# pananananas/MVD

Measured on AMD Instinct MI355X. Metric: UNet forward-passes/sec @512x512 SD2.1+MV adapter, higher is better.
Workload: dtype bf16; 1 GPU; cfg4: configs[3]/[4]: 8 objects x 4 target views per GPU (32 pairs), camera FiLM + cross-view adapter; pairs_per_gpu=32, global_pairs=32, latent=64x64x4, image=512x512, forward=cold, hip_graph=False, q2_statistics=replica-local, parallelism=dp1 (pairs sharded by object), weights=synthetic seeded, SD2.1 shapes (865.9M UNet x2 + 99.2M adapter + 19.1M camera), encoder_weights=distinct

## Files before the change

include/mvd_hip.h:

```cpp
#ifndef MVD_HIP_H
#define MVD_HIP_H
#include <stddef.h>
#include <stdint.h>

#ifdef __cplusplus
extern "C" {
#endif

#define MVD_MAX_LEVELS 4

typedef struct {
  int in_channels;
  int out_channels;
  int num_levels;
  int block_out_channels[MVD_MAX_LEVELS];
  int num_heads[MVD_MAX_LEVELS];
  int layers_per_block;
  int cross_attention_dim;
  int norm_num_groups;
  float norm_eps;
  int cam_output_dim;
  int cam_hidden_dim;
  int simple_cam_encoder;
  float cam_modulation_strength;
} mvd_config_t;

typedef struct mvd_engine mvd_engine_t;

const char* mvd_last_error(void);

int mvd_engine_create(const mvd_config_t* cfg, mvd_engine_t** out);
int mvd_engine_destroy(mvd_engine_t* e);

int mvd_engine_set_weight(mvd_engine_t* e, int set, const char* slot, const void* ptr, int64_t numel, int dtype);
int mvd_engine_clear_weights(mvd_engine_t* e, int set);

int64_t mvd_engine_workspace_bytes(mvd_engine_t* e, int batch, int height, int width, int text_len, int ref_batch);
int64_t mvd_engine_refcache_bytes(mvd_engine_t* e, int ref_batch, int height, int width, int keep_features);
int mvd_engine_bind_workspace(mvd_engine_t* e, void* ws, int64_t ws_bytes, void* refcache, int64_t refcache_bytes);

enum {
  MVD_USE_CAMERA = 1,
  MVD_USE_IMAGE = 2,
  MVD_REUSE_REF = 4,
  MVD_KEEP_FEATURES = 8,
  MVD_SHARE_REF = 16,
  MVD_DEEPCACHE_REFRESH = 32,
  MVD_DEEPCACHE_SHALLOW = 64
};


typedef struct {
  int batch;
  int height, width;
  int text_len;
  const float* sample;
  const float* timesteps;
  const float* text;
  const float* source_camera;
  const float* target_camera;
  int cam_rows;
  int cam_batch;
  const float* fourier_proj;
  const float* source_latents;
  const float* encoder_text;
  int ref_batch;
  int flags;
  float* out;
// ... 22 lines not shown

int mvd_engine_set_deepcache(mvd_engine_t* e, int branch);
int mvd_engine_clear_deepcache(mvd_engine_t* e);
int64_t mvd_engine_deepcache_bytes(mvd_engine_t* e, int batch, int height, int width);
int mvd_engine_bind_deepcache(mvd_engine_t* e, void* ptr, int64_t bytes);

int mvd_engine_set_profiling(mvd_engine_t* e, int enable);
int mvd_engine_profile_summary(mvd_engine_t* e, int cap, int* cls, int* launches, double* ms, double* flops, double* bytes);
int mvd_engine_profile_shapes(mvd_engine_t* e, char* buf_host, int cap);

int mvd_engine_num_features(mvd_engine_t* e);
int mvd_engine_feature_shape(mvd_engine_t* e, int idx, int* channels, int* height, int* width);
int mvd_engine_get_feature(mvd_engine_t* e, int idx, float* out_nchw, void* stream);
int mvd_engine_encode_cameras(mvd_engine_t* e, const float* source_camera, const float* target_camera, int cam_rows,
                              int batch, const float* fourier_proj, float* out_emb, void* stream);
int mvd_engine_apply_modulation(mvd_engine_t* e, const char* name, const float* emb, int batch, const float* x_nchw,
                                int channels, int hw, float* out_nchw, void* stream);
int mvd_engine_get_camera_embedding(mvd_engine_t* e, float* out, void* stream);
int mvd_engine_film_params(mvd_engine_t* e, const float* emb, int cam_batch, int out_rows, float* out, void* stream);
int mvd_engine_time_projection(mvd_engine_t* e, const float* timesteps, int batch, float* out, void* stream);

int mvd_op_linear(const void* a, const void* a2, int k1, int k2, const void* w, const float* bias, const float* rowvec,
                  int ld_rowvec, int rows_per_batch, const void* res, float alpha, int geglu, void* out, int out_f32,
                  int m, int n, int force_cfg, int splitk, float* splitk_ws ,
                  void* stream);
int mvd_op_linear_ld(const void* a, const void* a2, int k1, int k2, const void* w, int ldw, const float* bias, const float* rowvec,
                     int ld_rowvec, int rows_per_batch, const void* res, int ldres, float alpha, int geglu, void* out, int ldo,
                     int out_f32, int m, int n, int force_cfg, int splitk, float* splitk_ws ,
                     void* stream);
int mvd_op_ln_linear(const void* x, int k, const void* w_folded, const float* c1, const float* c2, float eps, int geglu,
                     void* out, int m, int n, void* stream);
int mvd_op_linear_xs(const void* x, int ldx, const void* w_packed, int m, int k, int units, int geglu, int ln, float ln_eps,
                     const void* res, int ldres, void* out, int ldo, int csplit, void* stream);
int mvd_op_conv3x3_ws(const void* x, int batch, int h, int w, int c, const void* w_packed, const float* bias, const float* rowvec,
                      int ld_rowvec, const void* res, const void* sc, const void* sc2, int sc_c1, int sc_c2, void* out, int n,
                      int variant, void* stream);
int mvd_op_conv3x3(const void* x, int batch, int in_h, int in_w, int cin, int stride, int upsample, int asym_pad, const void* w,
                   const float* bias, const float* rowvec, int ld_rowvec, const void* res, const void* sc, const void* sc2,
                   int sc_c1, int sc_c2, void* out, int cout, int force_cfg, int splitk, float* splitk_ws, void* stream);
int mvd_op_conv3x3_up4(const void* x, int batch, int in_h, int in_w, int cin, const void* w4, const float* bias, void* out, int cout,
                       int force_cfg, void* stream);
int mvd_op_attention(const void* q, const void* k, const void* v, void* o, int batch, int heads, int nq, int nk, int ldq,
                     int ldk, int ldv, int ldo, float scale, void* stream);
int mvd_op_attention_grouped(const void* q, const void* k, const void* v, void* o, int batch, int heads, int nq, int nk, int ldq,
                             int ldk, int ldv, int ldo, float scale, int kv_group, void* stream);
int mvd_op_attention_objects(const void* q, const void* k, const void* v, void* o, int batch, int heads, int nq, int nk, int ldq,
                             int ldk, int ldv, int ldo, float scale, int kv_group, int kv_objects, void* stream);
int mvd_op_attention_mapped(const void* q, const void* k, const void* v, void* o, int batch, int heads, int nq, int nk, int ldq,
                            int ldk, int ldv, int ldo, float scale, const int* kv_index_host, int kv_elements, void* stream);
int64_t mvd_op_attention_split_ws_bytes(int batch, int heads, int nq, int nsplit);
int mvd_op_attention_split(const void* q, const void* k, const void* v, void* o, int batch, int heads, int nq, int nk, int ldq,
                           int ldk, int ldv, int ldo, int nsplit, void* ws, void* stream);
int mvd_op_groupnorm(const void* x0, const void* x1, int c0, int c1, int batch, int hw, int groups, float eps,
                     const float* gamma, const float* beta, int silu, void* y, float* ws, void* stream);
int mvd_op_layernorm(const void* x, int rows, int c, float eps, const float* gamma, const float* beta, void* y,
                     void* stream);
int mvd_op_refnorm(const void* x, int batch, int hw, int c, void* y, void* stream);
int mvd_op_refnorm_grouped(const void* x, int batch, int group, int hw, int c, void* y, void* stream);
int mvd_op_film(const void* x, int batch, int hw, int c, const float* scale, const float* shift, void* y, void* stream);
int mvd_op_conv_in(const void* x, int batch, int h, int w, int cin, const float* wt, const float* bias, int cout, void* y,
                   void* stream);
int mvd_op_conv_out(const void* x, int batch, int h, int w, int c, const void* wt, const float* bias, int cout, float* y,
                    void* stream);
int mvd_op_nchw_to_nhwc(const float* x, int batch, int c, int hw, const float* scale, const float* shift, void* y,
                        void* stream);
int mvd_op_nhwc_to_nchw(const void* x, int batch, int hw, int c, float* y, void* stream);
int mvd_op_f32_to_bf16(const float* x, int64_t n, void* y, void* stream);
int mvd_op_skinny_linear(const float* x, int ldx, int batch, int k, const void* w, int wbf16, const float* bias, int n, int act_in,
                         float* y, int ldy, void* stream);
int mvd_op_timestep_embedding(const float* t, int batch, int dim, float* y, void* stream);
int mvd_op_camera_features(const float* src, const float* tgt, int batch, int cam_rows, int nfreq, float max_freq, float* rflat,
                           float* enc, void* stream);
int mvd_op_layernorm_f32(const float* x, int rows, int c, float eps, const float* gamma, const float* beta, int silu, int nseg,
                         float* y, void* stream);
int mvd_op_skinny_linear_grouped(const float* x, int ldx, int xseg, int batch, int k, const float* w, const float* bias, int n,
                                 const int* seg_end, int nseg, float* y, int ldy, void* stream);
int mvd_op_film_params(const float* raw, int batch, int dim, float strength, float* scale, float* shift, int out_rows,
                       void* stream);
int mvd_op_film_params_grouped(const float* raw, int batch, const int* seg_end, int nseg, float strength, float* out, int out_rows,
                               void* stream);
int mvd_op_im2col_in(const float* x, int batch, int c, int h, int w, const float* scale, const float* shift, int ld_ss, void* y,
                     void* stream);
int mvd_op_film_nchw_f32(const float* x, int batch, int c, int hw, const float* scale, const float* shift, float* y, void* stream);
int mvd_gemm_num_configs(void);
int mvd_debug_last_gemm_plan(int* out);
int mvd_debug_last_attention_plan(int* out);
int mvd_debug_last_groupnorm_plan(int* out);
long mvd_debug_up4_launches(void);
int mvd_debug_last_gemm_nowait(void);
int mvd_debug_pick_splitk(int m, int n, int k, int geglu);
int mvd_debug_pick_splitk_conv(int m, int n, int k);
int mvd_debug_dense_route(int m, int n, int k1, int k2, int* out);
int mvd_debug_gemm_pp_takes(int m, int n, int k, int ldw, int ldres, int ldo);
int mvd_gemm_sm_num_tiles(void);
int mvd_debug_set_attention_nw(int nw_log2);
int mvd_debug_ragged_tables(const int* view_counts, int objects, int g, int* adapter, int* text);
// ... 17 lines not shown
int mvd_op_vit_fold(const float* x, const float* delta, int64_t n, float* out, void* stream);
int mvd_op_clip_l2norm(float* x, int rows, int dim, void* stream);
int mvd_op_vae_pointwise(const float* x, int batch, int cin, int cout, int hw, const float* w, const float* bias, float* y, void* stream);
int64_t mvd_debug_clip_linear_ws_bytes(int M, int N, int K, int out_f32);
int mvd_debug_clip_linear(const void* a, int K, int M, const void* w, const float* bias, int N, void* out, int out_f32, void* ws,
                          int64_t ws_bytes, int* route_out, void* stream);
int mvd_debug_clip_attention(const void* qkv_bf16, void* out_bf16, int batch, int heads, int tokens, void* stream);
typedef enum {
  MVD_DBG_NO_SM_LN_FOLD = 1,
  MVD_DBG_SM_NO_SPLITK = 2,
  MVD_DBG_NO_SM = 4,
  MVD_DBG_NO_SPLIT_KV = 8,
  MVD_DBG_ONE_STREAM = 16,
  MVD_DBG_SINGLE_STREAM_POLICY = 32,
  MVD_DBG_SIDE_DEFAULT_PRIORITY = 64,
  MVD_DBG_NO_XS = 128,
  MVD_DBG_NO_WS = 256,
  MVD_DBG_WS_SMALL_MAPS = 512,
  MVD_DBG_WS_BLOCK64 = 1024,
  MVD_DBG_WS_NO_SHORTCUT = 2048,
  MVD_DBG_WS_NOT_IN_ENCODER = 4096,
  MVD_DBG_WS_ONLY_IN_ENCODER = 8192,
  MVD_DBG_WS_THEN_TILED = 16384,
  MVD_DBG_WS_CHECK = 32768,
  MVD_DBG_GRAPH_ONE_STREAM = 65536,
  MVD_DBG_PP_ROW_MAJOR = 131072,
  MVD_DBG_NO_DEEP_CONV_SPLIT = 262144,
  MVD_DBG_LATE_FROM_UP1 = 524288,
  MVD_DBG_NO_UP4 = 1048576,
  MVD_DBG_GN_ONE_PASS = 2097152,
  MVD_DBG_FORK_LATE = 4194304,
  MVD_DBG_SKINNY_VECTOR = 8388608
} mvd_debug_flag_t;
int mvd_debug_set_flags(int flags);

int mvd_op_ddpm_step(const float* model_out, const float* sample, const float* noise, float c0, float c1, float c2,
                     float c3, float sigma, float* out, int64_t n, void* stream);
int mvd_op_cfg_combine(const float* uncond_cond, float guidance_scale, float* out, int64_t n_half, void* stream);
int mvd_op_sampler_step(const float* model_out, int guided, float guidance_scale, const float* sample, const float* x0_prev,
                        const float* noise, float a0, float a1, float p, float q, float r, float sigma, float* out,
                        float* x0_out, int64_t n, void* stream);
int mvd_op_cfg_rescale(const float* uncond_cond, float guidance_scale, float guidance_rescale, float* out, int64_t rows,
                       int64_t n_row, void* stream);
int mvd_op_sampler_step_rescaled(const float* model_out, float guidance_scale, float guidance_rescale, const float* sample,
                                 const float* x0_prev, const float* noise, float a0, float a1, float p, float q, float r,
                                 float sigma, float* out, float* x0_out, int64_t rows, int64_t n_row, void* stream);
int mvd_debug_cfg_rescale_plan(int64_t n_row, int* out);
int mvd_op_apg(const float* uncond_cond, float guidance_scale, float eta, float norm_threshold, float momentum,
               float guidance_rescale, float* momentum_buffer, float* out, int64_t rows, int64_t n_row, void* stream);
int mvd_op_sampler_step_apg(const float* model_out, float guidance_scale, float eta, float norm_threshold, float momentum,
                            float guidance_rescale, int space, float* momentum_buffer, const float* sample, const float* x0_prev,
                            const float* noise, float a0, float a1, float p, float q, float r, float sigma, float* out,
                            float* x0_out, int64_t rows, int64_t n_row, void* stream);
int mvd_debug_apg_plan(int64_t n_row, int* out);

int mvd_op_freeu(const void* hidden, int C, const void* skip, int Cs, int B, int H, int W, float b, float s, void* hidden_out,
                 void* skip_out, void* stream);

int mvd_op_add_noise(const float* x0, const float* noise, const int32_t* timesteps, const float* sqrt_ac, const float* sqrt_1mac,
                     int num_train_timesteps, float* noisy, float* velocity, int batch, int64_t per_sample, void* stream);
int64_t mvd_op_noise_loss_ws_bytes(int batch, int64_t per_sample);
int mvd_op_noise_loss(const float* pred, const float* noise, const float* x0, const float* noisy, const int32_t* timesteps,
                      const float* sqrt_ac, const float* sqrt_1mac, const float* snr, int num_train_timesteps, int prediction_type,
                      float snr_gamma, float* denoised, float* result, int batch, int64_t per_sample, void* ws, int64_t ws_bytes,
                      void* stream);
int64_t mvd_op_image_metrics_ws_bytes(int n, int c, int h, int w, int want_ssim);
// ... 148 lines not shown
```

mvd_amd/_lib.py:

```python
from __future__ import annotations

import ctypes as C
import enum
import os

HERE = os.path.dirname(os.path.abspath(__file__))
LIB_PATH = os.environ.get("MVD_HIP_LIB") or os.path.join(HERE, "libmvd_hip.so")

MVD_MAX_LEVELS = 4
MVD_USE_CAMERA, MVD_USE_IMAGE, MVD_REUSE_REF, MVD_KEEP_FEATURES, MVD_SHARE_REF = 1, 2, 4, 8, 16
MVD_DEEPCACHE_REFRESH, MVD_DEEPCACHE_SHALLOW = 32, 64


class MvdError(RuntimeError):
    pass


class DebugFlag(enum.IntFlag):
    NO_SM_LN_FOLD = 1
    SM_NO_SPLITK = 2
    NO_SM = 4
    NO_SPLIT_KV = 8
    ONE_STREAM = 16
    SINGLE_STREAM_POLICY = 32
# ... 34 lines not shown
        ("norm_eps", C.c_float),
    ]


class mvd_text_config_t(C.Structure):
    _fields_ = [
        ("vocab_size", C.c_int), ("hidden_size", C.c_int), ("intermediate_size", C.c_int), ("num_layers", C.c_int),
        ("num_heads", C.c_int), ("max_positions", C.c_int), ("layer_norm_eps", C.c_float), ("act", C.c_int),
    ]


class mvd_vision_config_t(C.Structure):
    _fields_ = [
        ("image_size", C.c_int), ("patch_size", C.c_int), ("hidden_size", C.c_int), ("intermediate_size", C.c_int),
        ("num_layers", C.c_int), ("num_heads", C.c_int), ("projection_dim", C.c_int), ("layer_norm_eps", C.c_float), ("act", C.c_int),
    ]


class mvd_forward_args_t(C.Structure):
    _fields_ = [
        ("batch", C.c_int), ("height", C.c_int), ("width", C.c_int), ("text_len", C.c_int),
        ("sample", C.c_void_p), ("timesteps", C.c_void_p), ("text", C.c_void_p),
        ("source_camera", C.c_void_p), ("target_camera", C.c_void_p), ("cam_rows", C.c_int), ("cam_batch", C.c_int),
        ("fourier_proj", C.c_void_p), ("source_latents", C.c_void_p), ("encoder_text", C.c_void_p),
        ("ref_batch", C.c_int), ("flags", C.c_int), ("out", C.c_void_p), ("views", C.c_int),
    ]


_SIGS = {
    "mvd_last_error": (C.c_char_p, []),
    "mvd_engine_create": (C.c_int, [C.POINTER(mvd_config_t), C.POINTER(C.c_void_p)]),
    "mvd_engine_destroy": (C.c_int, [C.c_void_p]),
    "mvd_engine_set_weight": (C.c_int, [C.c_void_p, C.c_int, C.c_char_p, C.c_void_p, C.c_int64, C.c_int]),
    "mvd_engine_clear_weights": (C.c_int, [C.c_void_p, C.c_int]),
    "mvd_engine_workspace_bytes": (C.c_int64, [C.c_void_p, C.c_int, C.c_int, C.c_int, C.c_int, C.c_int]),
    "mvd_engine_workspace_bytes_args": (C.c_int64, [C.c_void_p, C.POINTER(mvd_forward_args_t)]),
    "mvd_engine_workspace_bytes_objects": (C.c_int64, [C.c_void_p, C.POINTER(mvd_forward_args_t), C.c_int]),
    "mvd_engine_refcache_bytes": (C.c_int64, [C.c_void_p, C.c_int, C.c_int, C.c_int, C.c_int]),
    "mvd_engine_bind_workspace": (C.c_int, [C.c_void_p, C.c_void_p, C.c_int64, C.c_void_p, C.c_int64]),
    "mvd_unet_forward": (C.c_int, [C.c_void_p, C.POINTER(mvd_forward_args_t), C.c_void_p]),
    "mvd_unet_forward_objects": (C.c_int, [C.c_void_p, C.POINTER(mvd_forward_args_t), C.c_int, C.c_void_p]),
    "mvd_unet_forward_ragged": (C.c_int, [C.c_void_p, C.POINTER(mvd_forward_args_t), C.POINTER(C.c_int), C.c_int, C.c_void_p]),
    "mvd_engine_workspace_bytes_ragged": (C.c_int64, [C.c_void_p, C.POINTER(mvd_forward_args_t), C.POINTER(C.c_int), C.c_int]),
    "mvd_debug_ragged_tables": (C.c_int, [C.POINTER(C.c_int), C.c_int, C.c_int, C.POINTER(C.c_int), C.POINTER(C.c_int)]),
    "mvd_engine_set_profiling": (C.c_int, [C.c_void_p, C.c_int]),
    "mvd_engine_profile_summary": (C.c_int, [C.c_void_p, C.c_int, C.POINTER(C.c_int), C.POINTER(C.c_int),
                                             C.POINTER(C.c_double), C.POINTER(C.c_double), C.POINTER(C.c_double)]),
    "mvd_engine_profile_shapes": (C.c_int, [C.c_void_p, C.c_char_p, C.c_int]),
    "mvd_engine_set_graph": (C.c_int, [C.c_void_p, C.c_int]),
    "mvd_engine_reference_pixels": (C.c_int64, [C.c_void_p, C.c_int, C.c_int]),
    "mvd_engine_reference_encode": (C.c_int, [C.c_void_p, C.POINTER(mvd_forward_args_t), C.c_void_p, C.c_void_p]),
    "mvd_engine_reference_finish": (C.c_int, [C.c_void_p, C.c_void_p, C.c_void_p]),
    "mvd_engine_share_encoder_weights": (C.c_int, [C.c_void_p, C.c_int]),
    "mvd_engine_num_features": (C.c_int, [C.c_void_p]),
    "mvd_engine_feature_shape": (C.c_int, [C.c_void_p, C.c_int, C.POINTER(C.c_int), C.POINTER(C.c_int), C.POINTER(C.c_int)]),
    "mvd_engine_get_feature": (C.c_int, [C.c_void_p, C.c_int, C.c_void_p, C.c_void_p]),
    "mvd_engine_encode_cameras": (C.c_int, [C.c_void_p, C.c_void_p, C.c_void_p, C.c_int, C.c_int, C.c_void_p, C.c_void_p, C.c_void_p]),
    "mvd_engine_apply_modulation": (C.c_int, [C.c_void_p, C.c_char_p, C.c_void_p, C.c_int, C.c_void_p, C.c_int, C.c_int, C.c_void_p, C.c_void_p]),
    "mvd_engine_get_camera_embedding": (C.c_int, [C.c_void_p, C.c_void_p, C.c_void_p]),
    "mvd_engine_film_params": (C.c_int, [C.c_void_p, C.c_void_p, C.c_int, C.c_int, C.c_void_p, C.c_void_p]),
    "mvd_engine_time_projection": (C.c_int, [C.c_void_p, C.c_void_p, C.c_int, C.c_void_p, C.c_void_p]),
    "mvd_op_linear": (C.c_int, [C.c_void_p, C.c_void_p, C.c_int, C.c_int, C.c_void_p, C.c_void_p, C.c_void_p, C.c_int,
                                C.c_int, C.c_void_p, C.c_float, C.c_int, C.c_void_p, C.c_int, C.c_int, C.c_int, C.c_int,
                                C.c_int, C.c_void_p, C.c_void_p]),
    "mvd_op_linear_ld": (C.c_int, [C.c_void_p, C.c_void_p, C.c_int, C.c_int, C.c_void_p, C.c_int, C.c_void_p, C.c_void_p, C.c_int,
                                   C.c_int, C.c_void_p, C.c_int, C.c_float, C.c_int, C.c_void_p, C.c_int, C.c_int, C.c_int, C.c_int,
                                   C.c_int, C.c_int, C.c_void_p, C.c_void_p]),
    "mvd_op_ln_linear": (C.c_int, [C.c_void_p, C.c_int, C.c_void_p, C.c_void_p, C.c_void_p, C.c_float, C.c_int, C.c_void_p,
                                   C.c_int, C.c_int, C.c_void_p]),
    "mvd_op_linear_xs": (C.c_int, [C.c_void_p, C.c_int, C.c_void_p, C.c_int, C.c_int, C.c_int, C.c_int, C.c_int, C.c_float,
                                   C.c_void_p, C.c_int, C.c_void_p, C.c_int, C.c_int, C.c_void_p]),
    "mvd_op_conv3x3_ws": (C.c_int, [C.c_void_p, C.c_int, C.c_int, C.c_int, C.c_int, C.c_void_p, C.c_void_p, C.c_void_p, C.c_int,
                                    C.c_void_p, C.c_void_p, C.c_void_p, C.c_int, C.c_int, C.c_void_p, C.c_int, C.c_int, C.c_void_p]),
    "mvd_op_conv3x3": (C.c_int, [C.c_void_p, C.c_int, C.c_int, C.c_int, C.c_int, C.c_int, C.c_int, C.c_int, C.c_void_p, C.c_void_p,
                                 C.c_void_p, C.c_int, C.c_void_p, C.c_void_p, C.c_void_p, C.c_int, C.c_int, C.c_void_p,
                                 C.c_int, C.c_int, C.c_int, C.c_void_p, C.c_void_p]),
    "mvd_op_attention": (C.c_int, [C.c_void_p, C.c_void_p, C.c_void_p, C.c_void_p, C.c_int, C.c_int, C.c_int, C.c_int,
                                   C.c_int, C.c_int, C.c_int, C.c_int, C.c_float, C.c_void_p]),
    "mvd_op_attention_grouped": (C.c_int, [C.c_void_p, C.c_void_p, C.c_void_p, C.c_void_p, C.c_int, C.c_int, C.c_int, C.c_int,
                                           C.c_int, C.c_int, C.c_int, C.c_int, C.c_float, C.c_int, C.c_void_p]),
    "mvd_op_attention_objects": (C.c_int, [C.c_void_p, C.c_void_p, C.c_void_p, C.c_void_p, C.c_int, C.c_int, C.c_int, C.c_int,
                                           C.c_int, C.c_int, C.c_int, C.c_int, C.c_float, C.c_int, C.c_int, C.c_void_p]),
    "mvd_op_attention_mapped": (C.c_int, [C.c_void_p, C.c_void_p, C.c_void_p, C.c_void_p, C.c_int, C.c_int, C.c_int, C.c_int,
                                          C.c_int, C.c_int, C.c_int, C.c_int, C.c_float, C.POINTER(C.c_int), C.c_int, C.c_void_p]),
    "mvd_debug_attention_mapped_grouped": (C.c_int, [C.c_void_p, C.c_void_p, C.c_void_p, C.c_void_p, C.c_int, C.c_int, C.c_int, C.c_int,
                                                     C.c_int, C.c_int, C.c_int, C.c_int, C.c_float, C.c_int, C.c_int, C.POINTER(C.c_int),
                                                     C.c_int, C.c_void_p]),
    "mvd_debug_attention_pair_ws_bytes": (C.c_int64, [C.POINTER(C.c_int), C.POINTER(C.c_int), C.POINTER(C.c_int), C.c_int, C.c_int,
                                                      C.c_float, C.c_int]),
    "mvd_debug_attention_pair": (C.c_int, [C.POINTER(C.c_void_p), C.POINTER(C.c_int), C.POINTER(C.c_int), C.POINTER(C.c_int), C.c_int,
                                           C.c_int, C.c_float, C.c_int, C.c_void_p, C.c_void_p]),
    "mvd_op_attention_split_ws_bytes": (C.c_int64, [C.c_int, C.c_int, C.c_int, C.c_int]),
    "mvd_op_attention_split": (C.c_int, [C.c_void_p, C.c_void_p, C.c_void_p, C.c_void_p, C.c_int, C.c_int, C.c_int, C.c_int, C.c_int,
                                         C.c_int, C.c_int, C.c_int, C.c_int, C.c_void_p, C.c_void_p]),
    "mvd_op_groupnorm": (C.c_int, [C.c_void_p, C.c_void_p, C.c_int, C.c_int, C.c_int, C.c_int, C.c_int, C.c_float,
                                   C.c_void_p, C.c_void_p, C.c_int, C.c_void_p, C.c_void_p, C.c_void_p]),
    "mvd_op_layernorm": (C.c_int, [C.c_void_p, C.c_int, C.c_int, C.c_float, C.c_void_p, C.c_void_p, C.c_void_p, C.c_void_p]),
    "mvd_op_refnorm": (C.c_int, [C.c_void_p, C.c_int, C.c_int, C.c_int, C.c_void_p, C.c_void_p]),
    "mvd_op_refnorm_grouped": (C.c_int, [C.c_void_p, C.c_int, C.c_int, C.c_int, C.c_int, C.c_void_p, C.c_void_p]),
    "mvd_op_film": (C.c_int, [C.c_void_p, C.c_int, C.c_int, C.c_int, C.c_void_p, C.c_void_p, C.c_void_p, C.c_void_p]),
    "mvd_op_conv_in": (C.c_int, [C.c_void_p, C.c_int, C.c_int, C.c_int, C.c_int, C.c_void_p, C.c_void_p, C.c_int, C.c_void_p, C.c_void_p]),
    "mvd_op_conv_out": (C.c_int, [C.c_void_p, C.c_int, C.c_int, C.c_int, C.c_int, C.c_void_p, C.c_void_p, C.c_int, C.c_void_p, C.c_void_p]),
    "mvd_op_nchw_to_nhwc": (C.c_int, [C.c_void_p, C.c_int, C.c_int, C.c_int, C.c_void_p, C.c_void_p, C.c_void_p, C.c_void_p]),
    "mvd_op_nhwc_to_nchw": (C.c_int, [C.c_void_p, C.c_int, C.c_int, C.c_int, C.c_void_p, C.c_void_p]),
    "mvd_op_f32_to_bf16": (C.c_int, [C.c_void_p, C.c_int64, C.c_void_p, C.c_void_p]),
    "mvd_op_skinny_linear": (C.c_int, [C.c_void_p, C.c_int, C.c_int, C.c_int, C.c_void_p, C.c_int, C.c_void_p, C.c_int, C.c_int,
                                        C.c_void_p, C.c_int, C.c_void_p]),
    "mvd_op_timestep_embedding": (C.c_int, [C.c_void_p, C.c_int, C.c_int, C.c_void_p, C.c_void_p]),
    "mvd_op_camera_features": (C.c_int, [C.c_void_p, C.c_void_p, C.c_int, C.c_int, C.c_int, C.c_float, C.c_void_p, C.c_void_p, C.c_void_p]),
    "mvd_op_layernorm_f32": (C.c_int, [C.c_void_p, C.c_int, C.c_int, C.c_float, C.c_void_p, C.c_void_p, C.c_int, C.c_int, C.c_void_p,
                                       C.c_void_p]),
    "mvd_op_skinny_linear_grouped": (C.c_int, [C.c_void_p, C.c_int, C.c_int, C.c_int, C.c_int, C.c_void_p, C.c_void_p, C.c_int,
                                               C.POINTER(C.c_int), C.c_int, C.c_void_p, C.c_int, C.c_void_p]),
    "mvd_op_film_params": (C.c_int, [C.c_void_p, C.c_int, C.c_int, C.c_float, C.c_void_p, C.c_void_p, C.c_int, C.c_void_p]),
    "mvd_op_film_params_grouped": (C.c_int, [C.c_void_p, C.c_int, C.POINTER(C.c_int), C.c_int, C.c_float, C.c_void_p, C.c_int, C.c_void_p]),
    "mvd_op_im2col_in": (C.c_int, [C.c_void_p, C.c_int, C.c_int, C.c_int, C.c_int, C.c_void_p, C.c_void_p, C.c_int, C.c_void_p, C.c_void_p]),
    "mvd_op_film_nchw_f32": (C.c_int, [C.c_void_p, C.c_int, C.c_int, C.c_int, C.c_void_p, C.c_void_p, C.c_void_p, C.c_void_p]),
    "mvd_gemm_num_configs": (C.c_int, []),
    "mvd_debug_last_gemm_plan": (C.c_int, [C.POINTER(C.c_int)]),
    "mvd_debug_up4_launches": (C.c_long, []),
    "mvd_op_conv3x3_up4": (C.c_int, [C.c_void_p, C.c_int, C.c_int, C.c_int, C.c_int, C.c_void_p, C.c_void_p, C.c_void_p, C.c_int, C.c_int,
                                     C.c_void_p]),
    "mvd_debug_last_gemm_nowait": (C.c_int, []),
    "mvd_debug_last_attention_plan": (C.c_int, [C.POINTER(C.c_int)]),
    "mvd_debug_last_groupnorm_plan": (C.c_int, [C.POINTER(C.c_int)]),
    "mvd_debug_pick_splitk": (C.c_int, [C.c_int, C.c_int, C.c_int, C.c_int]),
    "mvd_debug_pick_splitk_conv": (C.c_int, [C.c_int, C.c_int, C.c_int]),
    "mvd_debug_dense_route": (C.c_int, [C.c_int, C.c_int, C.c_int, C.c_int, C.POINTER(C.c_int)]),
    "mvd_debug_gemm_pp_takes": (C.c_int, [C.c_int, C.c_int, C.c_int, C.c_int, C.c_int, C.c_int]),
    "mvd_gemm_sm_num_tiles": (C.c_int, []),
    "mvd_debug_set_attention_nw": (C.c_int, [C.c_int]),
    "mvd_debug_set_flags": (C.c_int, [C.c_int]),
    "mvd_op_ddpm_step": (C.c_int, [C.c_void_p, C.c_void_p, C.c_void_p, C.c_float, C.c_float, C.c_float, C.c_float,
                                   C.c_float, C.c_void_p, C.c_int64, C.c_void_p]),
# ... 224 lines not shown
```

mvd_amd/csrc/engine.hip:

```cpp
#include <math.h>
#include <stdio.h>
#include <stdlib.h>
#include <string.h>

#include <mutex>
#include <string>
#include <unordered_map>
#include <vector>

#include "host_util.h"
#include "ragged.h"

int mvd_launch_silu_to_bf16(const float* x, int64_t n, bf16_t* y, hipStream_t s);

static int g_debug_flags = 0;
extern "C" int mvd_debug_set_flags(int flags) { g_debug_flags = flags; return 0; }
int mvd_debug_flags() { return g_debug_flags; }

namespace {

struct FeatureInfo { std::string name; int level; int C; int heads; std::string key;  };
constexpr int MVD_REF_ONLY_INTERNAL = 1 << 30;

}
// ... 7 lines not shown
  std::vector<FeatureInfo> feats;
  std::vector<bf16_t*> refkv;
  std::vector<bf16_t*> feat_keep;
  int rc_batch = 0, rc_h = 0, rc_w = 0; bool rc_valid = false; bool rc_keep = false;
  std::vector<int> rc_layout;
  float* ref_stats_out = nullptr;
  bool rc_pending = false;
  int64_t ref_pixels(int h, int w) const { int64_t n = 0; for (auto& f : feats) n += (int64_t)(h >> f.level) * (w >> f.level); return n; }
  int64_t feat_pixel_off(int idx) const { int64_t n = 0; for (int i = 0; i < idx; ++i) n += (int64_t)(rc_h >> feats[i].level) * (rc_w >> feats[i].level); return n; }
  float* cam_emb = nullptr; int cam_batch = 0;
  unsigned int* cnt_base = nullptr; int cnt_used = 0, cnt_cap = 0;
  hipStream_t side = nullptr;
  std::vector<hipEvent_t> feat_ev;
  hipEvent_t fork_ev = nullptr, join_ev = nullptr;
  bool dual_now = false;
  int ensure_side_stream() {
    if (side) return 0;
    {
      int lo = 0, hi = 0;
      (void)hipDeviceGetStreamPriorityRange(&lo, &hi);
      const int pr = (g_debug_flags & MVD_DBG_SIDE_DEFAULT_PRIORITY) ? 0 : hi;
      if (hipStreamCreateWithPriority(&side, hipStreamNonBlocking, pr) != hipSuccess) { mvd_set_error("engine: hipStreamCreate failed"); return -3; }
    }
    feat_ev.resize(feats.size());
    for (auto& ev : feat_ev) if (hipEventCreateWithFlags(&ev, hipEventDisableTiming) != hipSuccess) { mvd_set_error("engine: hipEventCreate failed"); return -3; }
    if (hipEventCreateWithFlags(&fork_ev, hipEventDisableTiming) != hipSuccess || hipEventCreateWithFlags(&join_ev, hipEventDisableTiming) != hipSuccess) { mvd_set_error("engine: hipEventCreate failed"); return -3; }
    return 0;
  }
  bool share_encoder = false;
  bool freeu_on = false; float freeu_b[2] = {1.f, 1.f}, freeu_s[2] = {1.f, 1.f};
  bool dc_on = false; int dc_branch = 0;
  void* dc_ptr = nullptr; int64_t dc_bytes = 0;
  uint64_t weight_gen = 0;
  struct DeepRecord { bool valid = false; int batch = 0, h = 0, w = 0, cam = 0, img = 0, branch = 0; uint64_t wgen = 0; std::vector<int> layout; } dc_rec;
  bool dc_sizing = false;
  int dc_hidden_channels() const { return cfg.layers_per_block - 1 - dc_branch >= 1 ? cfg.block_out_channels[0] : cfg.block_out_channels[1]; }
  struct HostState {
    std::vector<bf16_t*> refkv, feat_keep;
    int rc_batch, rc_h, rc_w; bool rc_valid, rc_keep;
    float* cam_emb; int cam_batch;
    std::vector<int> rc_layout;
  };
  HostState host_state() const { return {refkv, feat_keep, rc_batch, rc_h, rc_w, rc_valid, rc_keep, cam_emb, cam_batch, rc_layout}; }
  void set_host_state(const HostState& h) {
    refkv = h.refkv; feat_keep = h.feat_keep; rc_batch = h.rc_batch; rc_h = h.rc_h; rc_w = h.rc_w; rc_valid = h.rc_valid;
    rc_keep = h.rc_keep; cam_emb = h.cam_emb; cam_batch = h.cam_batch; rc_layout = h.rc_layout;
  }
  struct GraphEntry { std::string key; hipGraph_t g; hipGraphExec_t x; HostState after; };
  bool dual_late = false;
  bool graph_on = false;
  std::vector<GraphEntry> graphs;
  std::vector<std::string> graph_seen;
  void drop_graphs() {
    for (auto& ge : graphs) { (void)hipGraphExecDestroy(ge.x); (void)hipGraphDestroy(ge.g); }
    graphs.clear(); graph_seen.clear();
  }
  struct KvSlot { std::vector<int> layout , host ; int* dev = nullptr; uint64_t used = 0; };
  static constexpr size_t KV_SLOTS = 8;
  std::vector<KvSlot> kv_slots; uint64_t kv_tick = 0;
  ~mvd_engine() {
    drop_graphs();
    for (auto& sl : kv_slots) if (sl.dev) (void)hipFree(sl.dev);
    for (hipEvent_t ev : ev_pool) (void)hipEventDestroy(ev);
    for (hipEvent_t ev : feat_ev) if (ev) (void)hipEventDestroy(ev);
    if (fork_ev) (void)hipEventDestroy(fork_ev);
    if (join_ev) (void)hipEventDestroy(join_ev);
    if (side) (void)hipStreamDestroy(side);
  }
  std::vector<int> temb_off;
  int temb_total = 0;
  std::vector<int> tkv_off;
  int tkv_total = 0;
  bool prof = false;
  bool prof_overlap = false;
  struct ProfRec { int cls; double flops; double bytes; hipEvent_t e0, e1; int M, N, K, tag; };
  int prof_M = 0, prof_N = 0, prof_K = 0, prof_tag = 0;
  std::vector<ProfRec> prof_recs;
  std::vector<hipEvent_t> ev_pool; size_t ev_used = 0;
  hipEvent_t get_event() {
    if (ev_used == ev_pool.size()) { hipEvent_t ev = nullptr; (void)hipEventCreate(&ev); ev_pool.push_back(ev); }
    return ev_pool[ev_used++];
  }
};

static inline int gemm_class(const MvdGemmArgs& g, int cfg, int splitk) {
  if (cfg == 8) return MVD_PC_GEMM_128X320;
  if (cfg == 7) return splitk > 1 ? MVD_PC_PP_SPLITK : (g.seg[0].mode == MVD_A_CONV3 ? MVD_PC_PP_CONV3 : (g.ln_c1 ? MVD_PC_PP_LN_DENSE : MVD_PC_PP_DENSE));
  return MVD_PC_GEMM_256X160 + cfg;
}
int mvd_attention_pick_nw(const MvdAttnArgs& a);

namespace {

#ifdef MVD_PROBE
struct WsCheckRec { std::string slot; int set; bool side; const char* p[4]; size_t n[4]; };
// ... 107 lines not shown
      if (sm_S > 1) {
        g.splitk = sm_S; g.splitk_nowait = nowait ? 1 : 0; g.part = talloc<float>((size_t)sm_S * g.M * g.N);
        const int tiles = ((g.M + 63) / 64) * (g.N / 64);
        g.tile_cnt = e->cnt_base + e->cnt_used;
        e->cnt_used += tiles;
        if (!dry && e->cnt_used > e->cnt_cap) { mvd_set_error("forward: split-K tile counters exhausted (%d > %d)", e->cnt_used, e->cnt_cap); return err = -15; }
      }
      int r = 0;
      if (!dry) {
        const double fl = 2.0 * g.M * (double)g.N * g.Ktot;
        e->prof_M = g.M; e->prof_N = g.N; e->prof_K = g.Ktot; e->prof_tag = (tag_base >= 0 ? tag_base : g.seg[0].mode * 100 + g.geglu * 10) + (sm_S > 1 ? sm_S : 0);
        r = profiled(MVD_PC_SM_64X64 + sm_tile, fl, 0.0, [&] { return mvd_launch_gemm_sm(g, s, sm_tile, sm_ns); });
      }
      e->tmp.off = mark;
      return r;
    }
    int S = 1, fc = -1;
    tiled_plan(g, S, fc);
    const size_t mark = e->tmp.off;
    if (S > 1) { g.splitk = S; g.part = talloc<float>((size_t)S * g.M * g.N); } else g.splitk = 1;
    static const bool trace = MVD_ENV_INT("MVD_TRACE_GEMM", 0) != 0;
    if (trace && !dry) fprintf(stderr, "gemm M=%d N=%d K=%d mode=%d nseg=%d geglu=%d cfg=%d splitk=%d\n", g.M, g.N, g.Ktot, g.seg[0].mode, g.nseg, g.geglu, mvd_gemm_pick_config(g), S);
    int r = 0;
    if (!dry) {
      const double fl = 2.0 * g.M * (double)g.N * g.Ktot;
      e->prof_M = g.M; e->prof_N = g.N; e->prof_K = g.Ktot; e->prof_tag = (tag_base >= 0 ? tag_base : g.seg[0].mode * 100 + g.geglu * 10) + (S > 1 ? S : 0);
      r = launch_tiled(g, s, fc, [&](auto&& launch) { return profiled(e->prof ? gemm_class(g, mvd_gemm_pick_config(g), S) : 0, fl, 0.0, launch); });
    }
    e->tmp.off = mark;
    return r;
  }

  int try_xs(const bf16_t* x, int K, int M, const std::string& slot, int64_t n_full, int N, bool geglu, bool ln,
             const bf16_t* res, int ldres, void* out, int ldo, int set_override = -1) {
    if (err) return err;
    if (dry || (g_debug_flags & MVD_DBG_NO_XS) || K != 320 || slot.empty() || !has(slot, set_override)) return 0;
    MvdXsArgs a; memset(&a, 0, sizeof(a));
    a.x = x; a.ldx = K; a.M = M; a.K = K; a.units = N / 32; a.geglu = geglu; a.ln = ln; a.ln_eps = 1e-5f;
    a.res = res; a.ldres = ldres; a.out = (bf16_t*)out; a.ldo = ldo;
    if (N % 64 || !mvd_gemm_xs_applicable(a)) return 0;
    if ((long)((M + 255) / 256) * mvd_gemm_xs_pick_csplit(a) < 448) return 0;
    a.w = WB(slot, (n_full / 32) * 21 * 512, set_override);
    if (!a.w) return err;
    e->prof_M = M; e->prof_N = N; e->prof_K = K; e->prof_tag = geglu * 10 + (ln ? 1 : 0);
    const int r = profiled(geglu ? MVD_PC_XS_GEGLU : (res ? MVD_PC_XS_RESIDUAL : (ln ? MVD_PC_XS_LN_DENSE : MVD_PC_XS_DENSE)), 2.0 * M * (double)N * K, 0.0, [&] { return mvd_launch_gemm_xs(a, s); });
    return r ? r : 1;
  }

  int linear(const bf16_t* a, const bf16_t* a2, int k1, int k2, int M, const bf16_t* w, const float* bias, int N,
             const bf16_t* res, int ldres, void* out, int ldo, bool geglu = false, bool out_f32 = false, int ldw = 0,
             const std::string& xs = std::string(), int xs_set = -1) {
    if (!xs.empty() && !a2 && !k2 && !geglu && !out_f32) {
      const int r = try_xs(a, k1, M, xs, N, N, false, false, res, ldres, out, ldo, xs_set);
      if (r) return r < 0 ? r : 0;
    }
    MvdGemmArgs g = gemm_dense(a, a2, k1, k2, M, w, ldw, bias, N, out, ldo);
    g.res = res; g.ldres = ldres; g.geglu = geglu; g.out_f32 = out_f32;
    return gemm(g);
  }

  int ln_linear(const bf16_t* x, int M, int C, const std::string& ln_key, const std::string& slot, int64_t n_full, int N,
                const float* bias, bf16_t* ln_tmp, void* out, int ldo, bool geglu) {
    MvdGemmArgs g = gemm_dense(x, nullptr, C, 0, M, nullptr, 0, nullptr, N, out, ldo);
    g.geglu = geglu;
    {
      const int r = try_xs(x, C, M, slot + ".wx", n_full, N, geglu, true, nullptr, 0, out, ldo);
      if (r) return r < 0 ? r : 0;
    }
    static const bool use_fold = MVD_ENV_INT("MVD_LN_FOLD", 1) != 0;
    auto sm_fold_ok = [&]() {
      MvdGemmArgs t = g;
      static const float dummy = 0.f;
      t.ln_c1 = &dummy; t.bias = &dummy; t.W = reinterpret_cast<const bf16_t*>(&dummy);
      int a_, b_, c_;
      return sm_enabled() && !(g_debug_flags & MVD_DBG_NO_SM_LN_FOLD) && mvd_gemm_sm_plan(t, &a_, &b_, &c_);
    };
// ... 248 lines not shown
      const bf16_t* kv2 = tkv + c.e->tkv_off[feat_idx];
      const int ldkv = c.e->tkv_total;
      CHECK(c.ln_linear(h, M, C, key + ".ln2", key + ".attn2.q", (int64_t)(packed ? 2 : 1) * C, nq, nullptr, ln, q2, nq, false));
      MvdAttnArgs a; memset(&a, 0, sizeof(a));
      a.batch = B_; a.heads = heads; a.scale = scale; a.prescaled = 1; a.nprob = ad ? 2 : 1;
      a.p[0] = {q2, kv2, kv2 + C, o_self, nq, ldkv, ldkv, C, (int64_t)hw * nq, (int64_t)L * ldkv, (int64_t)L * ldkv, (int64_t)hw * C, hw, L};
      if (ad) a.p[1] = {q2 + C, rkv + 2 * C, rkv + 3 * C, o_ref, nq, 4 * C, 4 * C, C, (int64_t)hw * nq, (int64_t)ref_nk * 4 * C, (int64_t)ref_nk * 4 * C, (int64_t)hw * C, hw, ref_nk};
      if (ad) o.layout->fill_map(false, &a.kv_group[0], &a.kv_objects[0], &a.kv_index[0]);
      if (ad) o.layout->fill_map(true, &a.kv_group[1], &a.kv_objects[1], &a.kv_index[1]);
      CHECK(c.attention(a));
      CHECK(c.linear(o_self, o_ref, C, ad ? C : 0, M, c.WB(key + ".attn2.out.w", (int64_t)C * ld_out), c.WF(key + ".attn2" + bias_slot, C), C, h, C, h, C, false, false, ld_out,
                     ad ? std::string() : key + ".attn2.out.wx"));
    }
    {
      bf16_t* ff = c.talloc<bf16_t>((size_t)M * 4 * C);
      CHECK(c.ln_linear(h, M, C, key + ".ln3", key + ".ff1", (int64_t)8 * C, 8 * C, c.WF(key + ".ff1.b", 8 * C), ln, ff, 4 * C, true));
      const bool tail = c.has(key + ".tail.w");
      if (tail || c.dry) {
        c.tag_base = 50;
        const int r = c.linear(ff, h, 4 * C, C, M, c.WB(key + ".tail.w", (int64_t)C * 5 * C), c.WF(key + ".tail.b", C), C, x.p, C, out.p, C);
        c.tag_base = -1;
        CHECK(r);
      }
      if (!tail) {
        CHECK(c.linear(ff, nullptr, 4 * C, 0, M, c.WB(key + ".ff2.w", (int64_t)C * 4 * C), c.WF(key + ".ff2.b", C), C, h, C, h, C));
        CHECK(c.linear(h, nullptr, C, 0, M, c.WB(key + ".proj_out.w", (int64_t)C * C), c.WF(key + ".proj_out.b", C), C, x.p, C, out.p, C, false, false, 0, key + ".proj_out.wx"));
      }
    }
    c.e->tmp.off = mark;

    if (o.capture) {
      const size_t mk = c.e->tmp.off;
      bf16_t* rn = c.talloc<bf16_t>((size_t)M * C);
      if (o.defer_norm) {
        if (!c.dry && !c.err) CHECK(mvd_launch_refstats(out.p, B_, hw, C, o.stats + 2 * c.e->feat_pixel_off(feat_idx), c.s));
      } else {
        if (!c.dry && !c.err) CHECK(o.layout->per_object_stats() ? mvd_launch_refnorm_grouped(out.p, B_, 1, hw, C, rn, c.s) : mvd_launch_refnorm(out.p, B_, hw, C, rn, c.s));
        CHECK(c.linear(rn, nullptr, C, 0, M, c.WB(key + ".ref_kv.w", (int64_t)4 * C * C, 0), nullptr, 4 * C, nullptr, 0, c.e->refkv[feat_idx], 4 * C, false, false, 0,
                       key + ".ref_kv.wx", 0));
        if (c.e->dual_now && !c.dry && !c.err && hipEventRecord(c.e->feat_ev[feat_idx], c.s) != hipSuccess) { mvd_set_error("forward: hipEventRecord failed"); return -3; }
      }
      if (c.e->rc_keep && !c.dry && !c.err)
        CHECK((int)hipMemcpyAsync(c.e->feat_keep[feat_idx], out.p, (size_t)M * C * sizeof(bf16_t), hipMemcpyDeviceToDevice, c.s));
      c.e->tmp.off = mk;
    }
    ++feat_idx;
    return c.err;
  }

  int film(const std::string& name, const Act& x, Act& out) {
    auto it = o.film_ss->find(name);
    if (it == o.film_ss->end()) { out = x; return 0; }
    if (c.dry || c.err) return c.err;
    return mvd_launch_film(x.p, x.B, x.hw(), x.C, it->second.first, it->second.second, x.C, out.p, c.s);
  }

  int down_resnet_pos(int i, int j) const { return i * cfg.layers_per_block + j; }
  int mid_resnet_pos(int j) const { return cfg.num_levels * cfg.layers_per_block + j; }
  int up_resnet_pos(int i, int j) const { return cfg.num_levels * cfg.layers_per_block + 2 + i * (cfg.layers_per_block + 1) + j; }
  int down_feat_pos(int i, int j) const { return i * cfg.layers_per_block + j; }
  int mid_feat_pos() const { return (cfg.num_levels - 1) * cfg.layers_per_block; }
  int up_feat_pos(int i, int j) const { return (cfg.num_levels - 1) * cfg.layers_per_block + 1 + (i - 1) * (cfg.layers_per_block + 1) + j; }

  int run(const Act& x_in, float* out_nchw) {
    const int n = cfg.num_levels, Lb = cfg.layers_per_block;
    const int C0 = cfg.block_out_channels[0];
    const bool shallow = o.deep == MVD_DEEPCACHE_SHALLOW, refresh = o.deep == MVD_DEEPCACHE_REFRESH;
    const int j0 = Lb - 1 - o.deep_branch;
    std::vector<Act> skips;
    const int TB = text_rows > 0 ? text_rows : B;
    tkv = c.aalloc<bf16_t>((size_t)TB * L * c.e->tkv_total);
    CHECK(c.linear(text, nullptr, cfg.cross_attention_dim, 0, TB * L, c.WB("text_kv.w", (int64_t)c.e->tkv_total * cfg.cross_attention_dim), nullptr,
// ... 57 lines not shown
        if (refresh && i == n - 1 && j == j0 && !c.dry && !c.err)
          CHECK((int)hipMemcpyAsync(o.deep_buf, h.p, (size_t)h.rows() * h.C * sizeof(bf16_t), hipMemcpyDeviceToDevice, c.s));
        Act r = c.new_act(B, h.H, h.W, co, true);
        resnet_idx = up_resnet_pos(i, j);
        if (o.freeu && i < 2) {
          const size_t fm = c.e->tmp.off;
          Act hf = c.new_act(B, h.H, h.W, h.C, false), sf = c.new_act(B, skip.H, skip.W, skip.C, false);
          if (!c.dry && !c.err) CHECK(mvd_launch_freeu(h.p, h.C, skip.p, skip.C, B, h.H, h.W, c.e->freeu_b[i], c.e->freeu_s[i], hf.p, sf.p, c.s));
          CHECK(resnet(bk + ".resnets." + std::to_string(j), hf, &sf, co, r));
          c.e->tmp.off = fm;
        } else {
          CHECK(resnet(bk + ".resnets." + std::to_string(j), h, &skip, co, r));
        }
        h = r;
        if (i > 0) {
          Act t = c.new_act(B, h.H, h.W, co, true);
          feat_idx = up_feat_pos(i, j);
          CHECK(transformer(bk + ".attentions." + std::to_string(j), h, cfg.num_heads[n - 1 - i], t));
          h = t;
        }
      }
      if (i + 1 < n) {
        Act u = c.new_act(B, h.H * 2, h.W * 2, co, true);
        CHECK(c.conv3(h, 1, 1, c.WB(bk + ".up.w", (int64_t)co * 9 * co), c.WF(bk + ".up.b", co), nullptr, 0, nullptr, nullptr, nullptr, 0, 0, u, bk + ".up.ws", bk + ".up.w4"));
        h = u;
      }
      if (o.film) { Act res = h; CHECK(film("up_" + std::to_string(i), h, res)); h = res; }
    }
    if (out_nchw) {
      Act t = c.new_act(B, h.H, h.W, C0, false);
      CHECK(c.groupnorm(h.p, nullptr, C0, 0, B, h.hw(), cfg.norm_eps, c.WF("conv_norm_out.g", C0), c.WF("conv_norm_out.b", C0), 1, t.p));
      const bf16_t* wo = c.WB("conv_out.w", (int64_t)cfg.out_channels * 9 * C0);
      const float* bo = c.WF("conv_out.b", cfg.out_channels);
      if (!c.dry && !c.err) CHECK(mvd_launch_conv_out(t.p, B, h.H, h.W, C0, wo, bo, cfg.out_channels, out_nchw, c.s));
    }
    return c.err;
  }
};

int time_path(Ctx& c, const float* timesteps, int B, const float** tproj_out) {
  const mvd_config_t& cfg = c.e->cfg;
  const int C0 = cfg.block_out_channels[0], TD = 4 * C0;
  float* sinus = c.talloc<float>((size_t)B * C0);
  float* t1 = c.talloc<float>((size_t)B * TD);
  float* emb = c.talloc<float>((size_t)B * TD);
  bf16_t* act = c.talloc<bf16_t>((size_t)B * TD);
  float* tproj = c.aalloc<float>((size_t)B * c.e->temb_total);
  const bf16_t* w1 = c.WB("time.l1.w", (int64_t)TD * C0);
  const float* b1 = c.WF("time.l1.b", TD);
  const bf16_t* w2 = c.WB("time.l2.w", (int64_t)TD * TD);
  const float* b2 = c.WF("time.l2.b", TD);
  const bf16_t* wp = c.WB("temb_proj.w", (int64_t)c.e->temb_total * TD);
  const float* bp = c.WF("temb_proj.b", c.e->temb_total);
  *tproj_out = tproj;
  if (c.err) return c.err;
  if (c.dry) return 0;
  CHECK(mvd_launch_timestep_embedding(timesteps, B, C0, sinus, c.s));
  CHECK(mvd_launch_skinny_linear(sinus, C0, B, C0, w1, 1, b1, TD, 0, t1, TD, c.s));
  CHECK(mvd_launch_skinny_linear(t1, TD, B, TD, w2, 1, b2, TD, 1, emb, TD, c.s));
  CHECK(mvd_launch_silu_to_bf16(emb, (int64_t)B * TD, act, c.s));
  CHECK(c.linear(act, nullptr, TD, 0, B, wp, bp, c.e->temb_total, nullptr, 0, tproj, c.e->temb_total, false, true));
  return 0;
}

int camera_embed(Ctx& c, const float* src, const float* tgt, int cam_rows, const float* proj, int B, float* emb) {
  const mvd_config_t& cfg = c.e->cfg;
  const int D = cfg.cam_output_dim, Hd = cfg.cam_hidden_dim;
  const int nfreq = (D / 2) / 3, encd = 6 * nfreq;
  const bool simple = cfg.simple_cam_encoder != 0;
  float* rflat = c.talloc<float>((size_t)B * 9);
  float* enc = c.talloc<float>((size_t)B * encd);
  float* encp = c.talloc<float>((size_t)B * D);
  float* cat = c.talloc<float>((size_t)B * 2 * D);
  float* bufa = c.talloc<float>((size_t)B * (D > Hd ? D : Hd));
  float* bufb = c.talloc<float>((size_t)B * (D > Hd ? D : Hd));
  auto lin = [&](const std::string& k, const float* x, int ldx, int kin, int nout, float* y, int ldy) -> int {
    const float* w = c.WF("cam." + k + ".weight", (int64_t)nout * kin, 0);
    const float* b = c.WF("cam." + k + ".bias", nout, 0);
    if (c.err) return c.err; if (c.dry) return 0;
    return mvd_launch_skinny_linear(x, ldx, B, kin, w, 0, b, nout, 0, y, ldy, c.s);
  };
  auto lnorm = [&](const std::string& k, const float* x, int n, int silu, float* y) -> int {
    const float* g = c.WF("cam." + k + ".weight", n, 0);
    const float* b = c.WF("cam." + k + ".bias", n, 0);
    if (c.err) return c.err; if (c.dry) return 0;
    return mvd_launch_layernorm_f32(x, B, n, 1e-5f, g, b, silu, y, c.s);
  };
  if (!c.dry && !c.err) {
    CHECK(mvd_launch_camera_features(src, tgt, B, cam_rows, nfreq, 10.0f, rflat, enc, c.s));
    CHECK(mvd_launch_skinny_linear(enc, encd, B, encd, proj, 0, nullptr, D, 0, encp, D, c.s));
  }
  const char* encs[2] = {"rotation_encoder", "translation_encoder"};
  for (int t = 0; t < 2; ++t) {
    const std::string p = encs[t];
// ... 178 lines not shown
      for (size_t i = 0; i < e->feats.size(); ++i) {
        const int lv = e->feats[i].level;
        const size_t hw = (size_t)(H >> lv) * (Wd >> lv);
        e->refkv[i] = (bf16_t*)e->persist.alloc((size_t)a.ref_batch * hw * 4 * e->feats[i].C * sizeof(bf16_t));
        if (keep) e->feat_keep[i] = (bf16_t*)e->persist.alloc((size_t)a.ref_batch * hw * e->feats[i].C * sizeof(bf16_t));
      }
      if (e->persist.overflow()) { mvd_set_error("forward: reference cache too small (%zu > %zu bytes)", e->persist.high, e->persist.cap); return -4; }
      e->rc_keep = keep; e->rc_batch = a.ref_batch; e->rc_h = H; e->rc_w = Wd; e->rc_layout = lay.key();
      if (!dry) { e->rc_valid = false; e->rc_pending = false; }
    }
  }

  const bool dual = use_img && !reuse && !ref_only;
  e->dual_late = false;
  e->dual_now = dual && !dry && !(e->graph_on && (g_debug_flags & MVD_DBG_GRAPH_ONE_STREAM)) && (!e->prof || e->prof_overlap) && !(g_debug_flags & MVD_DBG_ONE_STREAM);
  const bool early = dual && (g_debug_flags & MVD_DBG_FORK_LATE);
  auto fork = [&]() -> int {
    if (!e->dual_now) return 0;
    CHECK(e->ensure_side_stream());
    if (hipEventRecord(e->fork_ev, s) != hipSuccess || hipStreamWaitEvent(e->side, e->fork_ev, 0) != hipSuccess) { mvd_set_error("forward: stream fork failed"); return -3; }
    return 0;
  };
  if (!early) CHECK(fork());

  std::unordered_map<std::string, std::pair<float*, float*>> film_ss;
  if (use_cam) CHECK(camera_path(c, a, film_ss));
  const float* tproj_main = nullptr;
  const float* tproj_enc = nullptr;
  if (early) {
    c.set = 0;
    CHECK(time_path(c, a.timesteps, B, &tproj_main));
    c.set = e->share_encoder ? 0 : 1;
    float* tz = c.aalloc<float>(a.ref_batch);
    if (!dry) CHECK((int)hipMemsetAsync(tz, 0, a.ref_batch * sizeof(float), s));
    CHECK(time_path(c, tz, a.ref_batch, &tproj_enc));
    c.set = 0;
    CHECK(fork());
  }

  if (use_img && !reuse) {
    if (dual) e->tmp.off = e->tmp.high;
    const size_t tm = e->tmp.off, am = e->act.off;
    if (e->dual_now) { c.s = e->side; c.nowait = true; }
    c.set = e->share_encoder ? 0 : 1;
    const int Br = a.ref_batch;
    const float* tproj = tproj_enc;
    if (!tproj) {
      float* tz = c.talloc<float>(Br);
      if (!dry) CHECK((int)hipMemsetAsync(tz, 0, Br * sizeof(float), c.s));
      CHECK(time_path(c, tz, Br, &tproj));
    }
    bf16_t* tx = c.aalloc<bf16_t>((size_t)Br * L * xd);
    Act xin = c.new_act(Br, H, Wd, 64, true);
    if (!dry && !c.err) {
      CHECK(mvd_launch_f32_to_bf16(a.encoder_text, (int64_t)Br * L * xd, tx, c.s));
      CHECK(mvd_launch_im2col_in(a.source_latents, Br, cfg.in_channels, H, Wd, nullptr, nullptr, 0, xin.p, c.s));
    }
    PassOpts po; po.capture = true; po.ref_batch = Br; po.layout = &lay;
    po.defer_norm = ref_only; po.stats = e->ref_stats_out;
    UNetPass pass{c, cfg, po, Br, H, Wd, L, tx, tproj};
    CHECK(pass.run(xin, nullptr));
    if (!dry) { e->rc_valid = !ref_only; e->rc_pending = ref_only; }
    if (dual) {
      e->tmp.off = e->tmp.high;
      if (e->dual_now && hipEventRecord(e->join_ev, e->side) != hipSuccess) { mvd_set_error("forward: hipEventRecord failed"); return -3; }
      c.s = s; c.nowait = false;
    } else {
      e->tmp.off = tm; e->act.off = am;
    }
  }
  if (ref_only) {
    if (c.err) return c.err;
    if (!dry && (e->tmp.high + e->act.high > (size_t)e->ws_bytes)) { mvd_set_error("reference_encode: workspace too small"); return -4; }
    return 0;
  }

  c.set = 0;
  const float* tproj = tproj_main;
  if (!tproj) CHECK(time_path(c, a.timesteps, B, &tproj));
  const int TB = lay.text_rows(B);
  bf16_t* tx = c.aalloc<bf16_t>((size_t)TB * L * xd);
  Act xin = c.new_act(B, H, Wd, 64, true);
  if (!dry && !c.err) {
// ... 61 lines not shown
}

extern "C" {

int mvd_engine_create(const mvd_config_t* cfg, mvd_engine_t** out) {
  if (!cfg || !out) { mvd_set_error("engine_create: null argument"); return -1; }
  if (cfg->num_levels < 2 || cfg->num_levels > MVD_MAX_LEVELS || cfg->layers_per_block < 1) { mvd_set_error("engine_create: unsupported topology"); return -1; }
  for (int i = 0; i < cfg->num_levels; ++i) {
    const int c = cfg->block_out_channels[i];
    if (c % 64 || c % cfg->norm_num_groups || cfg->num_heads[i] * 64 != c) { mvd_set_error("engine_create: level %d: channels %d must be a multiple of 64/groups with head_dim 64 (heads %d)", i, c, cfg->num_heads[i]); return -1; }
  }
  if (cfg->cross_attention_dim % 64) { mvd_set_error("engine_create: cross_attention_dim must be a multiple of 64"); return -1; }
  if (cfg->in_channels > 7 || cfg->out_channels > 8) { mvd_set_error("engine_create: in_channels must be <= 7 (9*Cin <= 64) and out_channels <= 8"); return -1; }
  mvd_engine* e = new mvd_engine();
  e->cfg = *cfg;
  e->feats = enumerate_features(*cfg);
  int off = 0;
  for (auto& r : enumerate_resnets(*cfg)) { e->temb_off.push_back(off); off += r.cout; }
  e->temb_total = off;
  off = 0;
  for (auto& f : e->feats) { e->tkv_off.push_back(off); off += 2 * f.C; }
  e->tkv_total = off;
  *out = e;
  return 0;
}

int mvd_engine_destroy(mvd_engine_t* e) { delete e; return 0; }

int mvd_engine_set_weight(mvd_engine_t* e, int set, const char* slot, const void* ptr, int64_t numel, int dtype) {
  if (e) e->drop_graphs();
  if (!e || set < 0 || set > 1 || !slot || !ptr || numel <= 0 || dtype < 0 || dtype > 1) { mvd_set_error("set_weight: bad argument"); return -1; }
  if ((uintptr_t)ptr & 15) { mvd_set_error("set_weight: '%s' must be 16-byte aligned", slot); return -1; }
  e->w[set].m[slot] = Weight{ptr, numel, dtype};
  ++e->weight_gen;
  return 0;
}
int mvd_engine_clear_weights(mvd_engine_t* e, int set) {
  if (e) e->drop_graphs();
  if (!e || set < 0 || set > 1) { mvd_set_error("clear_weights: bad argument"); return -1; }
  e->w[set].m.clear();
  ++e->weight_gen;
  return 0;
}

static void fill_dry_args(mvd_forward_args_t& a, int batch, int h, int w, int L, int ref_batch) {
  memset(&a, 0, sizeof(a));
  a.batch = batch; a.height = h; a.width = w; a.text_len = L; a.ref_batch = ref_batch; a.cam_rows = 4;
  a.flags = MVD_USE_CAMERA | (ref_batch > 0 ? MVD_USE_IMAGE : 0);
}

int64_t mvd_engine_workspace_bytes(mvd_engine_t* e, int batch, int height, int width, int text_len, int ref_batch) {
  if (!e) { mvd_set_error("workspace_bytes: null engine"); return -1; }
  mvd_forward_args_t a; fill_dry_args(a, batch, height, width, text_len, ref_batch);
  const mvd_engine::HostState before = e->host_state();
  int r = forward_impl(e, a, nullptr, true);
  e->set_host_state(before);
  if (r) return r;
  return (int64_t)(((e->act.high + 255) & ~size_t(255)) + e->tmp.high + 4096);
}

static ViewLayout uniform_layout(const mvd_forward_args_t* args, int objects) {
  return args ? ViewLayout::uniform(objects, args->views, args->flags & MVD_SHARE_REF) : ViewLayout();
}

static int64_t workspace_bytes_args(mvd_engine_t* e, const mvd_forward_args_t* args, const ViewLayout& lay) {
  if (!e || !args) { mvd_set_error("workspace_bytes_args: null argument"); return -1; }
// ... 662 lines not shown
  mvd_ragged_build_tables(view_counts, objects, g, adapter, text);
  if (mvd_attention_check_index(adapter, g * R, g * objects) || mvd_attention_check_index(text, g * R, g * objects)) return -1;
  return g * R;
}

int mvd_op_attention_split(const void* q, const void* k, const void* v, void* o, int batch, int heads, int nq, int nk, int ldq,
                           int ldk, int ldv, int ldo, int nsplit, void* ws, void* stream) {
  MvdAttnArgs a; memset(&a, 0, sizeof(a));
  a.nprob = 1; a.batch = batch; a.heads = heads; a.scale = 0.f; a.prescaled = 1;
  a.p[0] = {(const bf16_t*)q, (const bf16_t*)k, (const bf16_t*)v, (bf16_t*)o, ldq, ldk, ldv, ldo,
            (int64_t)nq * ldq, (int64_t)nk * ldk, (int64_t)nk * ldv, (int64_t)nq * ldo, nq, nk};
  if (nsplit > 1) {
    if (!ws) { mvd_set_error("op_attention_split: null workspace"); return -1; }
    const size_t pb = (mvd_attention_split_ws_bytes(a, nsplit) + 255) & ~size_t(255);
    a.nsplit = nsplit; a.split_ws = ws; a.split_cnt = reinterpret_cast<unsigned int*>(reinterpret_cast<char*>(ws) + pb);
    if (hipMemsetAsync(a.split_cnt, 0, (size_t)mvd_attention_split_counters(a) * 4, (hipStream_t)stream) != hipSuccess) { mvd_set_error("op_attention_split: hipMemsetAsync failed"); return -3; }
  }
  return mvd_launch_attention(a, (hipStream_t)stream);
}

int mvd_op_groupnorm(const void* x0, const void* x1, int c0, int c1, int batch, int hw, int groups, float eps,
                     const float* gamma, const float* beta, int silu, void* y, float* ws, void* stream) {
  return mvd_launch_groupnorm((const bf16_t*)x0, (const bf16_t*)x1, c0, c1, batch, hw, groups, eps, gamma, beta, silu, (bf16_t*)y, ws, (hipStream_t)stream);
}
int mvd_op_layernorm(const void* x, int rows, int c, float eps, const float* gamma, const float* beta, void* y, void* stream) {
  return mvd_launch_layernorm((const bf16_t*)x, rows, c, eps, gamma, beta, (bf16_t*)y, (hipStream_t)stream);
}
int mvd_op_refnorm(const void* x, int batch, int hw, int c, void* y, void* stream) {
  return mvd_launch_refnorm((const bf16_t*)x, batch, hw, c, (bf16_t*)y, (hipStream_t)stream);
}
int mvd_op_refnorm_grouped(const void* x, int batch, int group, int hw, int c, void* y, void* stream) {
  return mvd_launch_refnorm_grouped((const bf16_t*)x, batch, group, hw, c, (bf16_t*)y, (hipStream_t)stream);
}
int mvd_op_film(const void* x, int batch, int hw, int c, const float* scale, const float* shift, void* y, void* stream) {
  return mvd_launch_film((const bf16_t*)x, batch, hw, c, scale, shift, c, (bf16_t*)y, (hipStream_t)stream);
}
int mvd_op_conv_in(const void* x, int batch, int h, int w, int cin, const float* wt, const float* bias, int cout, void* y, void* stream) {
  return mvd_launch_conv_in((const bf16_t*)x, batch, h, w, cin, wt, bias, cout, (bf16_t*)y, (hipStream_t)stream);
}
int mvd_op_conv_out(const void* x, int batch, int h, int w, int c, const void* wt, const float* bias, int cout, float* y, void* stream) {
  return mvd_launch_conv_out((const bf16_t*)x, batch, h, w, c, (const bf16_t*)wt, bias, cout, y, (hipStream_t)stream);
}
int mvd_op_nchw_to_nhwc(const float* x, int batch, int c, int hw, const float* scale, const float* shift, void* y, void* stream) {
  return mvd_launch_nchw_to_nhwc(x, batch, c, hw, scale, shift, c, (bf16_t*)y, (hipStream_t)stream);
}
int mvd_op_nhwc_to_nchw(const void* x, int batch, int hw, int c, float* y, void* stream) {
  return mvd_launch_nhwc_to_nchw_f32((const bf16_t*)x, batch, hw, c, y, (hipStream_t)stream);
}
int mvd_op_f32_to_bf16(const float* x, int64_t n, void* y, void* stream) {
  return mvd_launch_f32_to_bf16(x, n, (bf16_t*)y, (hipStream_t)stream);
}
int mvd_op_skinny_linear(const float* x, int ldx, int batch, int k, const void* w, int wbf16, const float* bias, int n, int act_in,
                         float* y, int ldy, void* stream) {
  return mvd_launch_skinny_linear(x, ldx, batch, k, w, wbf16, bias, n, act_in, y, ldy, (hipStream_t)stream);
}
int mvd_op_timestep_embedding(const float* t, int batch, int dim, float* y, void* stream) {
  return mvd_launch_timestep_embedding(t, batch, dim, y, (hipStream_t)stream);
}
int mvd_op_camera_features(const float* src, const float* tgt, int batch, int cam_rows, int nfreq, float max_freq, float* rflat, float* enc,
                           void* stream) {
  return mvd_launch_camera_features(src, tgt, batch, cam_rows, nfreq, max_freq, rflat, enc, (hipStream_t)stream);
}
int mvd_op_layernorm_f32(const float* x, int rows, int c, float eps, const float* gamma, const float* beta, int silu, int nseg, float* y,
                         void* stream) {
  return mvd_launch_layernorm_f32(x, rows, c, eps, gamma, beta, silu, y, (hipStream_t)stream, nseg);
}
static int op_seg_table(const int* seg_end, int nseg, MvdSegTable* seg, const char* what) {
  if (!seg_end || nseg < 1 || nseg > 16) { mvd_set_error("%s: 1..16 segment ends", what); return -1; }
  memset(seg, 0, sizeof(*seg));
  seg->n = nseg;
  for (int g = 0; g < nseg; ++g) {
// ... 30 lines not shown
```

mvd_amd/csrc/gemm_xs.hip:

```cpp
#include <stdio.h>
#include <stdlib.h>
#include <string.h>
#include "../../include/mvd_hip.h"
#include "kernels.h"
#include "bufaddr.h"

namespace {

#define XS_WAIT_VM(n) asm volatile("s_waitcnt vmcnt(" #n ")" ::: "memory")

template <int KS, bool GEGLU, bool RES, bool LN>
__global__ __launch_bounds__(256, 2) void gemm_xs_kernel(const MvdXsArgs a) {
  constexpr int NW = 4, RT = 2, NS = GEGLU ? 2 : 3;
  constexpr int STG = GEGLU ? 8192 : 4096;
  constexpr int UNIT = (KS + 1) * 1024;
  constexpr int P = KS / NW;
  static_assert(KS % NW == 0 && !(GEGLU && RES) && !(RES && LN), "shape of the instantiations");
  constexpr int E = 2 * RT + (RES ? 2 * RT : 0);
  extern __shared__ __attribute__((aligned(16))) unsigned char smem[];
  const int lane = threadIdx.x & 63;
  const int wave = __builtin_amdgcn_readfirstlane(threadIdx.x >> 6);
  const int r = lane & 31, h = lane >> 5;
#ifdef XS_DBG
  constexpr int dbg = XS_DBG;
#else
  constexpr int dbg = 0;
#endif

  int rb, cp;
  if (a.csplit == 1) { rb = blockIdx.x; cp = 0; }
  else {
    const int per = 8 * a.csplit, g = blockIdx.x / per, rem = blockIdx.x - g * per;
    rb = g * 8 + (rem & 7); cp = rem >> 3;
  }
  if (rb * 256 >= a.M) return;
  const int upp = a.units / a.csplit;
  const int u0 = cp * upp, nit = upp;
  const int row_w = rb * 256 + wave * (RT * 32);

  const __amdgpu_buffer_rsrc_t rs_w = buf_rsrc(a.w, a.units * UNIT);
  auto issue_unit = [&](int it, int stage) {
    unsigned char* dst = smem + stage * UNIT;
    const unsigned so = (unsigned)(u0 + it) * (unsigned)UNIT;
    if (dbg & 4) return;
#pragma unroll
    for (int i = 0; i < P; ++i) dma16(rs_w, dst + (wave * P + i) * 1024, (unsigned)lane * 16u, so + (unsigned)((wave * P + i) * 1024));
    dma4(rs_w, dst + KS * 1024 + wave * 256, (unsigned)lane * 4u, so + (unsigned)(KS * 1024 + wave * 256));
  };
  issue_unit(0, 0);
  if (NS == 3 && nit > 1) issue_unit(1, 1);

  const __amdgpu_buffer_rsrc_t rs_x = buf_rsrc(a.x, (int)((size_t)a.M * a.ldx * 2));
  u32x4 x[RT][KS];
#pragma unroll
  for (int t = 0; t < RT; ++t) {
    const int vo = (row_w + t * 32 + r) * a.ldx * 2 + h * 16;
#pragma unroll
    for (int s = 0; s < KS; ++s) x[t][s] = (dbg & 8) ? u32x4{0x3f803f80u, 0x3f803f80u, 0x3f803f80u, 0x3f803f80u} : __builtin_amdgcn_raw_buffer_load_b128(rs_x, vo + s * 32, 0, 0);
  }
  if constexpr (LN) {
    const float invk = 1.f / (float)(KS * 16);
    const bf16x2 ones2 = __builtin_bit_cast(bf16x2, 0x3f803f80u);
#pragma unroll
    for (int t = 0; t < RT; ++t) {
      float sm = 0.f, sq = 0.f;
#pragma unroll
      for (int s = 0; s < KS; ++s) {
        const unsigned d[4] = {x[t][s].x, x[t][s].y, x[t][s].z, x[t][s].w};
#pragma unroll
        for (int e = 0; e < 4; ++e) {
          const bf16x2 v = __builtin_bit_cast(bf16x2, d[e]);
          sq = __builtin_amdgcn_fdot2_f32_bf16(v, v, sq, false);
          sm = __builtin_amdgcn_fdot2_f32_bf16(v, ones2, sm, false);
        }
      }
      sm += __shfl_xor(sm, 32); sq += __shfl_xor(sq, 32);
      const float mean = sm * invk;
      const float rstd = rsqrtf(fmaxf(sq * invk - mean * mean, 0.f) + a.ln_eps);
      const float nb = -mean * rstd;
#pragma unroll
      for (int s = 0; s < KS; ++s) {
        const unsigned d[4] = {x[t][s].x, x[t][s].y, x[t][s].z, x[t][s].w};
        x[t][s] = u32x4{pack2bf(fmaf(bflo(d[0]), rstd, nb), fmaf(bfhi(d[0]), rstd, nb)), pack2bf(fmaf(bflo(d[1]), rstd, nb), fmaf(bfhi(d[1]), rstd, nb)),
                        pack2bf(fmaf(bflo(d[2]), rstd, nb), fmaf(bfhi(d[2]), rstd, nb)), pack2bf(fmaf(bflo(d[3]), rstd, nb), fmaf(bfhi(d[3]), rstd, nb))};
      }
    }
  }
  const u32x4 one_frag = {h == 0 ? 0x3f803f80u : 0u, 0u, 0u, 0u};

  const __amdgpu_buffer_rsrc_t rs_o = buf_rsrc(a.out, (int)((size_t)a.M * a.ldo * 2));
  __amdgpu_buffer_rsrc_t rs_r = rs_o;
  if (RES) rs_r = buf_rsrc(a.res, (int)((size_t)a.M * a.ldres * 2));
  int vo_r[RT];
#pragma unroll
  for (int t = 0; t < RT; ++t) {
    vo_r[t] = RES ? (row_w + t * 32 + r) * a.ldres * 2 + h * 32 : 0;
  }

#ifdef XS_STAMPS
  long long st_acc[6] = {0, 0, 0, 0, 0, 0};
  const long long st_begin = (long long)__builtin_amdgcn_s_memtime();
  const long long st_rbegin = (long long)__builtin_amdgcn_s_memrealtime();
  long long st_t = st_begin;
#define XS_STAMP(i) do { const long long n_ = (long long)__builtin_amdgcn_s_memtime(); st_acc[i] += n_ - st_t; st_t = n_; } while (0)
#else
#define XS_STAMP(i) do {} while (0)
#endif
  float gs[16 * RT];

  auto top = [&](int it, int stage) {
    XS_STAMP(4);
    if (it == 0) XS_WAIT_VM(0);
    else if constexpr (GEGLU) { if ((it & 3) == 0) XS_WAIT_VM(8); else XS_WAIT_VM(0); }
    else if (it == nit - 1) { if (RES) XS_WAIT_VM(16); else XS_WAIT_VM(8); }
    else { if (RES) XS_WAIT_VM(22); else XS_WAIT_VM(14); }
    static_assert(P + 1 == 6 && 2 * E == (RES ? 16 : 8), "the counted waits above are written for these instantiations");
    __builtin_amdgcn_sched_barrier(0);
// ... 143 lines not shown
        f32x16 gg[RT];
        multiply(stage, gg, gs, false);
#pragma unroll
        for (int t = 0; t < RT; ++t)
#pragma unroll
          for (int q = 0; q < 16; ++q) gs[t * 16 + q] = gg[t][q];
        stage = stage == NS - 1 ? 0 : stage + 1;
      }
      {
        top(it + 1, stage);
        f32x16 acc[RT];
        multiply(stage, acc, gs, true);
#pragma unroll
        for (int t = 0; t < RT; ++t)
#pragma unroll
          for (int q = 0; q < 16; ++q) acc[t][q] *= gs[t * 16 + q];
        stage_tile((it >> 1) & 1, acc);
        if (it & 2) flush_group((u0 + it) >> 2);
        stage = stage == NS - 1 ? 0 : stage + 1;
      }
    }
  }
#ifdef XS_STAMPS
  XS_STAMP(4);
  if (wave == 0 && lane == 0) {
    asm volatile("s_waitcnt vmcnt(0)" ::: "memory");
    long long* dst = reinterpret_cast<long long*>(a.out + (size_t)a.M * a.ldo) + (size_t)blockIdx.x * 8;
    for (int i = 0; i < 5; ++i) dst[i] = st_acc[i];
    dst[5] = (long long)__builtin_amdgcn_s_memrealtime() - st_rbegin; dst[6] = (long long)__builtin_amdgcn_s_memtime() - st_begin; dst[7] = st_rbegin; (void)st_prolog;
  }
#endif
}

template <int KS, bool GEGLU, bool RES, bool LN>
int launch_xs(const MvdXsArgs& a, hipStream_t s) {
  constexpr int LDS_BYTES = (GEGLU ? 2 : 3) * (KS + 1) * 1024 + 4 * (GEGLU ? 8192 : 4096);
  static bool init[16] = {};
  int dev = 0;
  (void)hipGetDevice(&dev);
  if (!init[dev & 15]) {
    hipError_t e = hipFuncSetAttribute(reinterpret_cast<const void*>(&gemm_xs_kernel<KS, GEGLU, RES, LN>), hipFuncAttributeMaxDynamicSharedMemorySize, LDS_BYTES);
    if (e != hipSuccess) { mvd_set_error("gemm_xs: hipFuncSetAttribute: %s", hipGetErrorString(e)); return -2; }
    init[dev & 15] = true;
    if (MVD_ENV_INT("MVD_XS_TRACE", 0)) {
      int occ = -1;
      (void)hipOccupancyMaxActiveBlocksPerMultiprocessor(&occ, reinterpret_cast<const void*>(&gemm_xs_kernel<KS, GEGLU, RES, LN>), 256, LDS_BYTES);
      fprintf(stderr, "gemm_xs<%d,%d,%d,%d>: %d workgroups per CU by the occupancy query (LDS %d B)\n", KS, (int)GEGLU, (int)RES, (int)LN, occ, LDS_BYTES);
    }
  }
  const int nrb = (a.M + 255) / 256;
  const int grid = a.csplit == 1 ? nrb : ((nrb + 7) / 8) * 8 * a.csplit;
  g_mvd_last_gemm.cfg = 9; g_mvd_last_gemm.splitk = 1; g_mvd_last_gemm.tiles = nrb * a.csplit; g_mvd_last_gemm.grid = grid; g_mvd_last_gemm.per_cu = 2;
  hipLaunchKernelGGL((gemm_xs_kernel<KS, GEGLU, RES, LN>), dim3(grid), dim3(256), LDS_BYTES, s, a);
  hipError_t e = hipGetLastError();
  if (e != hipSuccess) { mvd_set_error("gemm_xs launch: %s", hipGetErrorString(e)); return -3; }
  return 0;
}

}

bool mvd_gemm_xs_applicable(const MvdXsArgs& a) {
  const size_t lim = (size_t)1 << 31;
  if (a.K != 320 || a.units <= 0 || a.M <= 0 || a.relu) return false;
  if (a.units % (a.geglu ? 4 : 2)) return false;
  if ((a.geglu || a.ln) && a.res) return false;
  if ((size_t)(a.M + 256) * a.ldx * 2 >= lim || (size_t)(a.M + 256) * a.ldo * 2 >= lim) return false;
  if (a.res && (size_t)(a.M + 256) * a.ldres * 2 >= lim) return false;
  if ((size_t)a.units * 21 * 1024 >= lim) return false;
  if ((a.ldx & 7) || (a.ldo & 7) || (a.res && (a.ldres & 7))) return false;
  return true;
}

int mvd_gemm_xs_pick_csplit(const MvdXsArgs& a) {
  const int nrb = (a.M + 255) / 256;
  const int groups = a.units / (a.geglu ? 4 : 2);
  int cs = 1;
  while (nrb * cs < 1024 && groups % (cs * 2) == 0 && groups / (cs * 2) >= 3) cs *= 2;
  return cs;
}

int mvd_launch_gemm_xs(const MvdXsArgs& a_in, hipStream_t s) {
  MvdXsArgs a = a_in;
  if (a.csplit <= 0) a.csplit = mvd_gemm_xs_pick_csplit(a);
  const int groups = a.units / (a.geglu ? 4 : 2);
  if (!mvd_gemm_xs_applicable(a) || groups % a.csplit) {
    mvd_set_error("gemm_xs: M=%d K=%d units=%d geglu=%d csplit=%d is not a shape of the X-stationary kernels", a.M, a.K, a.units, a.geglu, a.csplit);
    return -1;
  }
  if (a.geglu) return a.ln ? launch_xs<20, true, false, true>(a, s) : launch_xs<20, true, false, false>(a, s);
  if (a.res) return launch_xs<20, false, true, false>(a, s);
  return a.ln ? launch_xs<20, false, false, true>(a, s) : launch_xs<20, false, false, false>(a, s);
}

extern "C" int mvd_op_linear_xs(const void* x, int ldx, const void* w_packed, int m, int k, int units, int geglu, int ln, float ln_eps,
                                const void* res, int ldres, void* out, int ldo, int csplit, void* stream) {
  MvdXsArgs a; memset(&a, 0, sizeof(a));
  a.x = (const bf16_t*)x; a.ldx = ldx; a.w = (const bf16_t*)w_packed; a.M = m; a.K = k; a.units = units; a.geglu = geglu;
  a.ln = ln; a.ln_eps = ln_eps; a.res = (const bf16_t*)res; a.ldres = ldres; a.out = (bf16_t*)out; a.ldo = ldo; a.csplit = csplit;
  if (!x || !w_packed || !out) { mvd_set_error("mvd_op_linear_xs: null operand"); return -1; }
  return mvd_launch_gemm_xs(a, (hipStream_t)stream);
}
```

mvd_amd/csrc/kernels.h:

```cpp
#pragma once
#include <hip/hip_runtime.h>
#include <stdint.h>
#include <atomic>
#include "common.h"
#include "../../include/mvd_hip.h"

enum { MVD_A_DENSE = 0, MVD_A_CONV3 = 1 };

struct MvdASeg {
  const bf16_t* p0;
  const bf16_t* p1;
  int c0, c1;
  int mode;
  int ksize;
  int inH, inW;
  int stride;
  int ups;
  int asym;
};

struct MvdGemmArgs {
  MvdASeg seg[2];
  int nseg;
  const bf16_t* W;
// ... 22 lines not shown
  float ln_eps;
  int walk_cg;
};
static_assert(sizeof(MvdGemmArgs) == 280, "MvdGemmArgs is a kernel argument: a size change moves the hidden arguments of every GEMM kernel");

inline bool mvd_gemm_rowvec_aligned(const MvdGemmArgs& a) { return !a.rowvec || (a.ld_rowvec % 4 == 0 && ((uintptr_t)a.rowvec & 15) == 0); }
int mvd_launch_gemm(const MvdGemmArgs& a, hipStream_t s, int force_cfg = -1);
int mvd_gemm_pick_config(const MvdGemmArgs& a);
int mvd_launch_gemm_relu(const MvdGemmArgs& a, hipStream_t s, int cfg, bool glds);
int mvd_launch_splitk_reduce_relu(const MvdGemmArgs& a, hipStream_t s, int grid);
struct MvdLaunchPlan { int cfg, splitk, tiles, grid, per_cu, nowait; };
extern thread_local MvdLaunchPlan g_mvd_last_gemm;
extern std::atomic<long> g_mvd_up4_launches;
bool mvd_gemm_pp_applicable(const MvdGemmArgs& a);
bool mvd_gemm_pp_up4_applicable(const MvdGemmArgs& a);
int mvd_gemm_pp_walk(const MvdGemmArgs& a);
int mvd_debug_flags();
bool mvd_gemm_ln_fold_ok(const MvdGemmArgs& a);
int mvd_launch_gemm_pp(const MvdGemmArgs& a, hipStream_t s);
int mvd_launch_gemm_ring(const MvdGemmArgs& a, hipStream_t s);
bool mvd_gemm_sm_applicable(const MvdGemmArgs& a, int tile);
int mvd_launch_gemm_sm(const MvdGemmArgs& a, hipStream_t s, int tile, int nstage);
bool mvd_gemm_sm_plan(const MvdGemmArgs& a, int* tile, int* nstage, int* splitk);
struct MvdXsArgs {
  const bf16_t* x; int ldx;
  const bf16_t* w;
  int M, K, units;
  int geglu;
  int ln; float ln_eps;
  const bf16_t* res; int ldres;
  bf16_t* out; int ldo;
  int csplit;
  int relu;
};
bool mvd_gemm_xs_applicable(const MvdXsArgs& a);
int mvd_gemm_xs_pick_csplit(const MvdXsArgs& a);
int mvd_launch_gemm_xs(const MvdXsArgs& a, hipStream_t s);
struct MvdWsArgs {
  const bf16_t* x; int B, H, W, C;
  int ups;
  const bf16_t* sc0; const bf16_t* sc1; int scc0, scc1;
  const bf16_t* w;
  const float* bias;
  const float* rowvec; int ld_rowvec;
  const bf16_t* res; int ldres;
  bf16_t* out; int ldo;
  int M, N;
  int variant;
  int relu;
};
bool mvd_conv_ws_applicable(const MvdWsArgs& a);
size_t mvd_conv_ws_packed_elems(int C, int sc, int N);
int mvd_launch_conv_ws(const MvdWsArgs& a, hipStream_t s);
#define MVD_OP_SPLITK_COUNTERS 4096
int mvd_launch_splitk_reduce(const MvdGemmArgs& a, hipStream_t s);
int mvd_gemm_pick_splitk(const MvdGemmArgs& a);

struct MvdAttnProblem {
  const bf16_t* q; const bf16_t* k; const bf16_t* v; bf16_t* o;
  int ldq, ldk, ldv, ldo;
  int64_t bsq, bsk, bsv, bso;
  int nq, nk;
};
struct MvdAttnArgs {
  MvdAttnProblem p[2];
  int nprob;
  int batch, heads;
  float scale;
  int prescaled;
  int dbg;
  int nsplit;
  void* split_ws;
  unsigned int* split_cnt;
  int kv_group[2];
  int kv_objects[2];
  const int* kv_index[2];
};
int mvd_attention_check_index(const int* idx, int n, int elements);
int mvd_attention_pick_split(const MvdAttnArgs& a);
size_t mvd_attention_split_ws_bytes(const MvdAttnArgs& a, int nsplit);
int mvd_attention_split_counters(const MvdAttnArgs& a);
int mvd_launch_attention(const MvdAttnArgs& a, hipStream_t s);

#define MVD_GN_MAXCHUNK 256
int mvd_launch_groupnorm(const bf16_t* x0, const bf16_t* x1, int c0, int c1, int batch, int hw, int groups,
                         float eps, const float* gamma, const float* beta, int silu, bf16_t* y, float* ws,
                         hipStream_t s);
int mvd_launch_layernorm(const bf16_t* x, int rows, int c, float eps, const float* gamma, const float* beta,
                         bf16_t* y, hipStream_t s);
int mvd_launch_refnorm(const bf16_t* x, int batch, int hw, int c, bf16_t* y, hipStream_t s);
int mvd_launch_refnorm_grouped(const bf16_t* x, int batch, int group, int hw, int c, bf16_t* y, hipStream_t s);
int mvd_launch_refstats(const bf16_t* x, int batch, int hw, int c, float* stats , hipStream_t s);
int mvd_launch_refapply(const bf16_t* x, int batch, int hw, int c, const float* mean_k , bf16_t* y, hipStream_t s);

int mvd_launch_nchw_to_nhwc(const float* x, int batch, int c, int hw, const float* scale, const float* shift,
                            int ld_ss, bf16_t* y, hipStream_t s);
int mvd_launch_film(const bf16_t* x, int batch, int hw, int c, const float* scale, const float* shift, int ld_ss,
                    bf16_t* y, hipStream_t s);
int mvd_launch_freeu(const bf16_t* hidden, int C, const bf16_t* skip, int Cs, int B, int H, int W, float b, float s, bf16_t* hidden_out,
                     bf16_t* skip_out, hipStream_t stream);
int mvd_launch_conv_in(const bf16_t* x, int batch, int h, int w, int cin, const float* wt, const float* bias,
                       int cout, bf16_t* y, hipStream_t s);
int mvd_launch_conv_out(const bf16_t* x, int batch, int h, int w, int c, const bf16_t* wt, const float* bias,
                        int cout, float* y, hipStream_t s);
int mvd_launch_im2col_in(const float* x, int batch, int c, int h, int w, const float* scale, const float* shift, int ld_ss,
                         bf16_t* y, hipStream_t s);
int mvd_launch_f32_to_bf16(const float* x, int64_t n, bf16_t* y, hipStream_t s);
int mvd_launch_nhwc_to_nchw_f32(const bf16_t* x, int batch, int hw, int c, float* y, hipStream_t s);
int mvd_launch_maxpool2x2(const bf16_t* x, int batch, int h, int w, int c, bf16_t* y, hipStream_t s);

int mvd_launch_skinny_linear(const float* x, int ldx, int batch, int k, const void* w, int wbf16, const float* bias,
                             int n, int act_in, float* y, int ldy, hipStream_t s);
struct MvdSegTable { int n; int end[16]; };
int mvd_launch_skinny_linear_grouped(const float* x, int ldx, int xseg, int batch, int k, const float* w, const float* bias, int n,
                                     const MvdSegTable& seg, float* y, int ldy, hipStream_t s);
int mvd_launch_film_params_grouped(const float* raw, int batch, const MvdSegTable& seg, float strength, float* out, int out_rows,
                                   hipStream_t s);
int mvd_launch_layernorm_f32(const float* x, int rows, int c, float eps, const float* gamma, const float* beta,
                             int silu, float* y, hipStream_t s, int nseg = 1);
int mvd_launch_timestep_embedding(const float* t, int batch, int dim, float* y, hipStream_t s);
int mvd_launch_camera_features(const float* src, const float* tgt, int batch, int cam_rows, int nfreq,
                               float max_freq, float* rflat, float* enc, hipStream_t s);
int mvd_launch_film_params(const float* raw, int batch, int dim, float strength, float* scale, float* shift, int out_rows,
                           hipStream_t s);

int mvd_launch_film_nchw_f32(const float* x, int batch, int c, int hw, const float* scale, const float* shift, float* y,
                             hipStream_t s);

void mvd_set_error(const char* fmt, ...);

enum MvdProfClass {
  MVD_PC_GEMM_256X160 = 0, MVD_PC_GEMM_256X128 = 1, MVD_PC_GEMM_128X160 = 2, MVD_PC_GEMM_128X128 = 3, MVD_PC_GEMM_128X64 = 4,
  MVD_PC_GEMM_64X64 = 5,
  MVD_PC_PP_GEGLU = 6, MVD_PC_PP_DENSE = 7,
  MVD_PC_ATTN_1WAVE = 8, MVD_PC_ATTN_2WAVE = 9, MVD_PC_ATTN_4WAVE = 10, MVD_PC_ATTN_8WAVE = 11,
// ... 9 lines not shown
```

mvd_amd/csrc/misc.hip:

```cpp
#include <stdarg.h>
#include <stdio.h>
#include <stdlib.h>
#include "host_util.h"

static thread_local char g_err[512] = "";
void mvd_set_error(const char* fmt, ...) {
  va_list ap;
  va_start(ap, fmt);
  vsnprintf(g_err, sizeof(g_err), fmt, ap);
  va_end(ap);
}
extern "C" const char* mvd_last_error(void) { return g_err; }

namespace {

__global__ void nchw_to_nhwc_kernel(const float* __restrict__ x, int c, int hw, const float* __restrict__ scale,
                                    const float* __restrict__ shift, int ld_ss, bf16_t* __restrict__ y, long total) {
  const long i = (long)blockIdx.x * blockDim.x + threadIdx.x;
  if (i >= total) return;
  const int ch = i % c;
  const long bp = i / c;
  const int p = bp % hw;
  const int b = bp / hw;
  float v = x[((size_t)b * c + ch) * hw + p];
  if (scale) v = v * scale[(size_t)b * ld_ss + ch] + shift[(size_t)b * ld_ss + ch];
  y[i] = f2bf(v);
}

__global__ void nhwc_to_nchw_f32_kernel(const bf16_t* __restrict__ x, int hw, int c, float* __restrict__ y, long total) {
  const long i = (long)blockIdx.x * blockDim.x + threadIdx.x;
  if (i >= total) return;
  const int p = i % hw;
  const long bc = i / hw;
  const int ch = bc % c;
  const int b = bc / c;
  y[i] = bf2f(x[((size_t)b * hw + p) * c + ch]);
// ... 52 lines not shown
  const long pix = (long)blockIdx.x * 4 + (threadIdx.x >> 6);
  const int hw = h * w;
  if (pix >= (long)batch * hw) return;
  const int b = pix / hw, p = pix % hw;
  const int oy = p / w, ox = p % w;
  const int vec = c >> 3;
  float acc[8];
#pragma unroll
  for (int j = 0; j < 8; ++j) acc[j] = 0.f;
  for (int q = lane; q < 9 * vec; q += 64) {
    const int tap = q / vec, v = q % vec;
    const int iy = oy + tap / 3 - 1, ix = ox + tap % 3 - 1;
    if ((unsigned)iy >= (unsigned)h || (unsigned)ix >= (unsigned)w) continue;
    const u32x4 xv = *reinterpret_cast<const u32x4*>(x + ((size_t)b * hw + iy * w + ix) * c + v * 8);
#pragma unroll
    for (int co = 0; co < 8; ++co) {
      if (co < cout) {
        const u32x4 wv = *reinterpret_cast<const u32x4*>(wt + ((size_t)co * 9 + tap) * c + v * 8);
        float a = acc[co];
#pragma unroll
        for (int j = 0; j < 4; ++j) {
          a = fmaf(bflo(xv[j]), bflo(wv[j]), a);
          a = fmaf(bfhi(xv[j]), bfhi(wv[j]), a);
        }
        acc[co] = a;
      }
    }
  }
#pragma unroll
  for (int co = 0; co < 8; ++co) {
    if (co < cout) {
      const float t = wave_sum(acc[co]);
      if (lane == 0) y[((size_t)b * cout + co) * hw + p] = t + bias[co];
    }
  }
}

__global__ void f32_to_bf16_kernel(const float* __restrict__ x, long n, bf16_t* __restrict__ y) {
  for (long i = (long)blockIdx.x * blockDim.x + threadIdx.x; i < n; i += (long)gridDim.x * blockDim.x) y[i] = f2bf(x[i]);
}

template <bool WBF16>
__global__ __launch_bounds__(256) void skinny_linear_kernel(const float* __restrict__ x, int ldx, int batch, int k,
                                                             const void* __restrict__ wv, const float* __restrict__ bias,
                                                             int n, int act_in, float* __restrict__ y, int ldy) {
  constexpr int BC = 32;
  const int lane = threadIdx.x & 63;
  const int o = blockIdx.x * 4 + (threadIdx.x >> 6);
  if (o >= n) return;
  const bool vec = !WBF16 && (k & 3) == 0 && (ldx & 3) == 0;
  for (int b0 = 0; b0 < batch; b0 += BC) {
    float acc[BC];
#pragma unroll
    for (int j = 0; j < BC; ++j) acc[j] = 0.f;
    if (vec) {
      const float* wr = reinterpret_cast<const float*>(wv) + (size_t)o * k;
      for (int kk = lane * 4; kk < k; kk += 256) {
        const f32x4 w4 = *reinterpret_cast<const f32x4*>(wr + kk);
#pragma unroll
        for (int j = 0; j < BC; ++j) {
          if (b0 + j < batch) {
            f32x4 x4 = *reinterpret_cast<const f32x4*>(x + (size_t)(b0 + j) * ldx + kk);
            if (act_in == 1) { x4[0] = silu_f(x4[0]); x4[1] = silu_f(x4[1]); x4[2] = silu_f(x4[2]); x4[3] = silu_f(x4[3]); }
            acc[j] = fmaf(x4[0], w4[0], fmaf(x4[1], w4[1], fmaf(x4[2], w4[2], fmaf(x4[3], w4[3], acc[j]))));
          }
        }
// ... 324 lines not shown
      hipLaunchKernelGGL(word_sum_kernel, dim3(1024), dim3(256), 0, s, reinterpret_cast<const unsigned*>(y), (long)on, dsum + 1);
      hipLaunchKernelGGL(word_sum_kernel, dim3(1024), dim3(256), 0, s, reinterpret_cast<const unsigned*>(y1), (long)on, dsum + 2);
      unsigned long long hs[3] = {0, 0, 0};
      (void)hipMemcpyAsync(hs, dsum, sizeof(hs), hipMemcpyDeviceToHost, s);
      (void)hipStreamSynchronize(s);
      fprintf(stderr, "conv_out hash pid %d: input %016llx  out(4-pixel) %016llx  out(1-pixel, same input) %016llx\n", (int)getpid(), hs[0], hs[1], hs[2]);
    }
    if (MVD_ENV_INT("MVD_CONV_OUT_CMP", 0)) {
      static unsigned long long* cnt = nullptr; static float* yb = nullptr; static float* yr = nullptr; static size_t yn = 0;
      static unsigned long long seen[3] = {0, 0, 0}; static int calls = 0;
      const size_t on = (size_t)batch * cout * h * w;
      if (!cnt) { (void)hipHostMalloc(&cnt, 4 * sizeof(unsigned long long), hipHostMallocMapped); cnt[0] = cnt[1] = cnt[2] = cnt[3] = 0; }
      if (yn < on) { if (yb) { (void)hipFree(yb); (void)hipFree(yr); } (void)hipMalloc(&yb, on * sizeof(float)); (void)hipMalloc(&yr, on * sizeof(float)); yn = on; }
      hipLaunchKernelGGL(conv_out4_kernel, dim3(nblk(quads, 4)), dim3(256), 0, s, x, batch, h, w, c, wt, bias, cout, yb);
      hipLaunchKernelGGL(conv_out_kernel, dim3(nblk((long)batch * h * w, 4)), dim3(256), 0, s, x, batch, h, w, c, wt, bias, cout, yr);
      hipLaunchKernelGGL(conv_out_cmp_kernel, dim3(256), dim3(256), 0, s, y, yb, yr, (long)on, 1e-3f, cnt);
      ++calls;
      volatile unsigned long long* vc = cnt;
      const unsigned long long c0 = vc[0], c1 = vc[1], c2 = vc[2];
      if (c0 != seen[0] || c1 != seen[1] || c2 != seen[2] || calls == 2 || calls == 20) {
        seen[0] = c0; seen[1] = c1; seen[2] = c2;
        fprintf(stderr, "conv_out cmp pid %d after ~%d calls: first!=second %llu  |first-ref|>1e-3 %llu  |second-ref|>1e-3 %llu  last idx %llu (x mod 4 = %llu)\n",
                (int)getpid(), calls - 1, c0, c1, c2, (unsigned long long)vc[3], (unsigned long long)vc[3] % 4);
      }
    }
    return launch_check("conv_out4");
  }
#endif
  const long pix = (long)batch * h * w;
  hipLaunchKernelGGL(conv_out_kernel, dim3(nblk(pix, 4)), dim3(256), 0, s, x, batch, h, w, c, wt, bias, cout, y);
  return launch_check("conv_out");
}

int mvd_launch_f32_to_bf16(const float* x, int64_t n, bf16_t* y, hipStream_t s) {
  if (!x || !y || n <= 0) { mvd_set_error("f32_to_bf16: bad arguments"); return -1; }
  int grid = nblk(n, 256);
  if (grid > 4096) grid = 4096;
  hipLaunchKernelGGL(f32_to_bf16_kernel, dim3(grid), dim3(256), 0, s, x, (long)n, y);
  return launch_check("f32_to_bf16");
}

int mvd_launch_skinny_linear(const float* x, int ldx, int batch, int k, const void* w, int wbf16, const float* bias, int n,
                             int act_in, float* y, int ldy, hipStream_t s) {
  if (!x || !w || !y || batch <= 0 || batch > 4096 || k <= 0 || n <= 0 || ldx < k || ldy < n) { mvd_set_error("skinny_linear: bad arguments"); return -1; }
  const int kv = wbf16 ? 8 : 4;
  const bool vec = (k % kv) == 0 && (ldx % 4) == 0 && (((uintptr_t)x | (uintptr_t)w) & 15) == 0;
  static const int use_vec = MVD_ENV_INT("MVD_SKINNY_VEC", 1);
  if (vec && batch >= 8 && !(mvd_debug_flags() & MVD_DBG_SKINNY_VECTOR)) {
    const MvdSegTable none{};
    if (wbf16) hipLaunchKernelGGL((skinny_mfma_kernel<true, false>), dim3(nblk(n, 32)), dim3(256), 0, s, x, ldx, batch, k, w, bias, n, act_in, y, ldy, none, 0);
    else hipLaunchKernelGGL((skinny_mfma_kernel<false, false>), dim3(nblk(n, 32)), dim3(256), 0, s, x, ldx, batch, k, w, bias, n, act_in, y, ldy, none, 0);
    return launch_check("skinny_mfma");
  }
  if (vec && use_vec) {
    constexpr int F = 2;
    const dim3 g(nblk(n, 4 * F));
    if (wbf16) hipLaunchKernelGGL((skinny_linear_vec_kernel<true, F>), g, dim3(256), 0, s, x, ldx, batch, k, w, bias, n, act_in, y, ldy);
    else hipLaunchKernelGGL((skinny_linear_vec_kernel<false, F>), g, dim3(256), 0, s, x, ldx, batch, k, w, bias, n, act_in, y, ldy);
    return launch_check("skinny_linear");
  }
  if (wbf16) hipLaunchKernelGGL(skinny_linear_kernel<true>, dim3(nblk(n, 4)), dim3(256), 0, s, x, ldx, batch, k, w, bias, n, act_in, y, ldy);
  else hipLaunchKernelGGL(skinny_linear_kernel<false>, dim3(nblk(n, 4)), dim3(256), 0, s, x, ldx, batch, k, w, bias, n, act_in, y, ldy);
  return launch_check("skinny_linear");
}

int mvd_launch_skinny_linear_grouped(const float* x, int ldx, int xseg, int batch, int k, const float* w, const float* bias, int n,
// ... 86 lines not shown
```

mvd_amd/csrc/norm.hip:

```cpp
#include <stdlib.h>
#include "kernels.h"
#include "bufaddr.h"

namespace {

MVD_DEVINL void unpack8(const u32x4 v, float* f) {
  f[0] = bflo(v[0]); f[1] = bfhi(v[0]); f[2] = bflo(v[1]); f[3] = bfhi(v[1]);
  f[4] = bflo(v[2]); f[5] = bfhi(v[2]); f[6] = bflo(v[3]); f[7] = bfhi(v[3]);
}
MVD_DEVINL u32x4 pack8(const float* f) {
  return u32x4{pack2bf(f[0], f[1]), pack2bf(f[2], f[3]), pack2bf(f[4], f[5]), pack2bf(f[6], f[7])};
}

__global__ void gn_stats_kernel(const bf16_t* __restrict__ x0, const bf16_t* __restrict__ x1, int c0, int c1, int hw,
                                int groups, int rows_per_chunk, int R, float* __restrict__ ws) {
  extern __shared__ __attribute__((aligned(16))) float sh[];
  const int C = c0 + c1, vec = C >> 3;
  const int b = blockIdx.y, chunk = blockIdx.x, nchunk = gridDim.x;
  const int v = threadIdx.x % vec, r = threadIdx.x / vec;
  const int row0 = chunk * rows_per_chunk;
  const int row1 = min(hw, row0 + rows_per_chunk);
  const int ch = v * 8;
  const bool first = ch < c0;
  const bf16_t* src = first ? x0 + (size_t)b * hw * c0 + ch : x1 + (size_t)b * hw * c1 + (ch - c0);
// ... 347 lines not shown
    if (lane == 0) red[wave] = v;
    __syncthreads();
    return red[0] + red[1] + red[2] + red[3];
  };
  float s = 0.f;
  for (int e = threadIdx.x; e < total; e += 256) {
    const int b = e / vec, v = e % vec;
    float f[8];
    unpack8(*reinterpret_cast<const u32x4*>(x + ((size_t)b * hw + p) * c + v * 8), f);
#pragma unroll
    for (int j = 0; j < 8; ++j) s += f[j];
  }
  const float n = (float)group * (float)c;
  const float mean = block_sum(s) / n;
  float q = 0.f;
  for (int e = threadIdx.x; e < total; e += 256) {
    const int b = e / vec, v = e % vec;
    float f[8];
    unpack8(*reinterpret_cast<const u32x4*>(x + ((size_t)b * hw + p) * c + v * 8), f);
#pragma unroll
    for (int j = 0; j < 8; ++j) { const float d = f[j] - mean; q = fmaf(d, d, q); }
  }
  const float var = block_sum(q) / (n - 1.0f);
  const float k = 0.5f / fmaxf(sqrtf(var), 1e-6f);
  for (int e = threadIdx.x; e < total; e += 256) {
    const int b = e / vec, v = e % vec;
    float f[8];
    const size_t off = ((size_t)b * hw + p) * c + v * 8;
    unpack8(*reinterpret_cast<const u32x4*>(x + off), f);
#pragma unroll
    for (int j = 0; j < 8; ++j) f[j] = (f[j] - mean) * k;
    *reinterpret_cast<u32x4*>(y + off) = pack8(f);
  }
}

__global__ __launch_bounds__(256) void refstats_kernel(const bf16_t* __restrict__ x, int batch, int hw, int c, float* __restrict__ stats) {
  __shared__ float red[8];
  const int p = blockIdx.x;
  const int vec = c >> 3;
  const int total = batch * vec;
  const int lane = threadIdx.x & 63, wave = threadIdx.x >> 6;
  auto block_sum = [&](float v) -> float {
    v = wave_sum(v);
    __syncthreads();
    if (lane == 0) red[wave] = v;
    __syncthreads();
    return red[0] + red[1] + red[2] + red[3];
  };
  float s = 0.f;
  for (int e = threadIdx.x; e < total; e += 256) {
    const int b = e / vec, v = e % vec;
    float f[8];
    unpack8(*reinterpret_cast<const u32x4*>(x + ((size_t)b * hw + p) * c + v * 8), f);
#pragma unroll
    for (int j = 0; j < 8; ++j) s += f[j];
  }
  const float mean = block_sum(s) / ((float)batch * (float)c);
  float q = 0.f;
  for (int e = threadIdx.x; e < total; e += 256) {
    const int b = e / vec, v = e % vec;
    float f[8];
    unpack8(*reinterpret_cast<const u32x4*>(x + ((size_t)b * hw + p) * c + v * 8), f);
#pragma unroll
    for (int j = 0; j < 8; ++j) { const float d = f[j] - mean; q = fmaf(d, d, q); }
  }
  const float m2 = block_sum(q);
// ... 123 lines not shown
}

extern "C" int mvd_debug_last_groupnorm_plan(int* out) {
  if (!out) { mvd_set_error("last_groupnorm_plan: null argument"); return -1; }
  for (int i = 0; i < 6; ++i) out[i] = g_last_gn[i];
  return 0;
}

int mvd_launch_layernorm(const bf16_t* x, int rows, int c, float eps, const float* gamma, const float* beta, bf16_t* y,
                         hipStream_t s) {
  if (!x || !y || !gamma || !beta || rows <= 0 || c <= 0 || (c % 8) || c > 64 * 8 * 4) {
    mvd_set_error("layernorm: bad arguments rows=%d c=%d", rows, c);
    return -1;
  }
  const int grid = (rows + 3) / 4;
  if (c <= 512) hipLaunchKernelGGL(ln_kernel<1>, dim3(grid), dim3(256), 0, s, x, rows, c, eps, gamma, beta, y);
  else if (c <= 1024) hipLaunchKernelGGL(ln_kernel<2>, dim3(grid), dim3(256), 0, s, x, rows, c, eps, gamma, beta, y);
  else hipLaunchKernelGGL(ln_kernel<4>, dim3(grid), dim3(256), 0, s, x, rows, c, eps, gamma, beta, y);
  return check_launch("layernorm");
}

int mvd_launch_refstats(const bf16_t* x, int batch, int hw, int c, float* stats, hipStream_t s) {
  if (!x || !stats || batch <= 0 || hw <= 0 || c <= 0 || (c % 8)) { mvd_set_error("refstats: bad arguments"); return -1; }
  hipLaunchKernelGGL(refstats_kernel, dim3(hw), dim3(256), 0, s, x, batch, hw, c, stats);
  return check_launch("refstats");
}
int mvd_launch_refapply(const bf16_t* x, int batch, int hw, int c, const float* mean_k, bf16_t* y, hipStream_t s) {
  if (!x || !y || !mean_k || batch <= 0 || hw <= 0 || c <= 0 || (c % 8)) { mvd_set_error("refapply: bad arguments"); return -1; }
  const long total = (long)batch * hw * (c >> 3);
  long grid = (total + 255) / 256; if (grid > 4096) grid = 4096;
  hipLaunchKernelGGL(refapply_kernel, dim3((unsigned)grid), dim3(256), 0, s, x, batch, hw, c, mean_k, y);
  return check_launch("refapply");
}
int mvd_launch_refnorm(const bf16_t* x, int batch, int hw, int c, bf16_t* y, hipStream_t s) {
  if (!x || !y || batch <= 0 || hw <= 0 || c <= 0 || (c % 8)) { mvd_set_error("refnorm: bad arguments"); return -1; }
  hipLaunchKernelGGL(refnorm_kernel, dim3(hw), dim3(256), 0, s, x, batch, hw, c, y);
  return check_launch("refnorm");
}

int mvd_launch_refnorm_grouped(const bf16_t* x, int batch, int group, int hw, int c, bf16_t* y, hipStream_t s) {
  if (!x || !y || batch <= 0 || hw <= 0 || c <= 0 || (c % 8)) { mvd_set_error("refnorm_grouped: bad arguments"); return -1; }
  if (group <= 0 || batch % group) { mvd_set_error("refnorm_grouped: group %d does not divide the batch %d", group, batch); return -1; }
  if (batch / group > 65535) { mvd_set_error("refnorm_grouped: %d groups exceed the grid", batch / group); return -1; }
  hipLaunchKernelGGL(refnorm_grouped_kernel, dim3(hw, batch / group), dim3(256), 0, s, x, group, hw, c, y);
  return check_launch("refnorm_grouped");
}

int mvd_launch_layernorm_f32(const float* x, int rows, int c, float eps, const float* gamma, const float* beta, int silu,
                             float* y, hipStream_t s, int nseg) {
  if (!x || !y || !gamma || !beta || rows <= 0 || c <= 0 || nseg < 1) { mvd_set_error("layernorm_f32: bad arguments"); return -1; }
  hipLaunchKernelGGL(ln_f32_kernel, dim3(rows), dim3(256), 0, s, x, c, eps, gamma, beta, silu, y, nseg);
  return check_launch("layernorm_f32");
}
```

mvd_amd/distributed.py:

```python
from __future__ import annotations

import os
import socket
import time
from typing import Dict, Iterable, List, Sequence

import torch
import torch.distributed as dist


def init_from_env(backend: str = "nccl", set_device: bool = True) -> tuple:
    world = int(os.environ.get("WORLD_SIZE", "1"))
    rank = int(os.environ.get("RANK", "0"))
    local = int(os.environ.get("LOCAL_RANK", "0"))
    if set_device and backend == "nccl" and torch.cuda.is_available():
        torch.cuda.set_device(local)
    if world > 1 and not dist.is_initialized():
        os.environ.setdefault("MASTER_ADDR", "127.0.0.1")
        os.environ.setdefault("MASTER_PORT", "29500")
        kw = {}
        if backend == "nccl" and torch.cuda.is_available():
            kw["device_id"] = torch.device("cuda", local)
        dist.init_process_group(backend=backend, rank=rank, world_size=world, **kw)
    return rank, world, local
# ... 77 lines not shown
        bucket: List[torch.Tensor] = []
        size = 0

        def flush():
            nonlocal bucket, size, total, nb
            if not bucket:
                return
            flat = torch.cat([b.reshape(-1) for b in bucket])
            dist.broadcast(flat, src)
            off = 0
            for b in bucket:
                n = b.numel()
                b.copy_(flat[off:off + n].view_as(b))
                off += n
            total += flat.numel() * flat.element_size()
            nb += 1
            bucket, size = [], 0

        for t in ts:
            bucket.append(t)
            size += t.numel() * t.element_size()
            if size >= bucket_bytes:
                flush()
        flush()
    if tensors and tensors[0].is_cuda:
        torch.cuda.synchronize()
    return dict(bytes=total, seconds=time.perf_counter() - t0, buckets=nb)


def broadcast_engine_weights(engine, src: int = 0, bucket_bytes: int = 256 << 20) -> Dict[str, float]:
    if not dist.is_initialized() or dist.get_world_size() == 1:
        return dict(bytes=0, seconds=0.0, buckets=0)
    engine.consolidate_weights()
    return broadcast_arenas(engine._arenas.values(), src, bucket_bytes)


def merge_reference_stats(local: torch.Tensor, group=None) -> torch.Tensor:
    if local.dim() != 2 or local.shape[1] != 3:
        raise ValueError("merge_reference_stats expects [pixels][3] rows (n, mean, M2)")
    parts = [local]
    if dist.is_initialized() and dist.get_world_size(group) > 1:
        world = dist.get_world_size(group)
        on_host = local.is_cuda and dist.get_backend(group) == "gloo"
        src = local.cpu() if on_host else local.contiguous()
        parts = [torch.empty_like(src) for _ in range(world)]
        dist.all_gather(parts, src, group=group)
        parts = [p.to(local.device) for p in parts]
    return merge_stat_parts(parts)


def merge_stat_parts(parts: Sequence[torch.Tensor]) -> torch.Tensor:
    n = torch.zeros_like(parts[0][:, 0], dtype=torch.float64)
    mean = torch.zeros_like(n)
    m2 = torch.zeros_like(n)
    for p in parts:
        pn, pm, pq = p[:, 0].double(), p[:, 1].double(), p[:, 2].double()
        tot = n + pn
        delta = pm - mean
        mean = mean + delta * pn / tot
        m2 = m2 + pq + delta * delta * n * pn / tot
        n = tot
    mean, m2, n = mean.float(), m2.float(), n.float()
    k = 0.5 / (m2 / (n - 1.0)).sqrt().clamp_min(1e-6)
    return torch.stack([mean, k], dim=1).contiguous()


def any_rank(flag: bool, group=None, device=None) -> bool:
# ... 102 lines not shown
```

mvd_amd/engine.py:

```python
from __future__ import annotations

import ctypes as C
import os
from typing import Dict, List, Optional

import torch

from . import _lib as L
from .config import UNetConfig
from .layout import ViewLayout
from .packing import pack_camera, pack_unet


def _ptr(t: Optional[torch.Tensor]):
    return None if t is None else C.c_void_p(t.data_ptr())


class MVDEngine:
    def __init__(self, cfg: UNetConfig, cam_output_dim: int = 1024, cam_hidden_dim: int = 512,
                 simple_cam_encoder: bool = False, cam_modulation_strength: float = 0.2, device="cuda:0",
                 small_batch_twins: Optional[bool] = None, fold_tail: bool = True):
        if not torch.cuda.is_available():
            raise L.MvdError("MVDEngine needs a MI355X (torch.cuda.is_available() is False); there is no CPU fallback")
        self.cfg = cfg
# ... 46 lines not shown
            self._register(0, pack_unet(sd, self.cfg, self.device, adapter, ref_scale, self.small_batch_twins, self.fold_tail))

    def load_camera(self, sd: Dict[str, torch.Tensor]):
        with torch.no_grad():
            self._register(0, pack_camera(sd, self.device, len(self.cfg.block_out_channels)))

    def load_image_encoder(self, sd: Dict[str, torch.Tensor]):
        with torch.no_grad():
            self._register(1, pack_unet(sd, self.cfg, self.device, False, 0.0, self.small_batch_twins, self.fold_tail))
        self.share_encoder_weights(False)

    def share_encoder_weights(self, enable: bool = True):
        L.call("mvd_engine_share_encoder_weights", self._h, int(enable))
        if enable:
            L.call("mvd_engine_clear_weights", self._h, 1)
            self._weights[1] = {}
            self._arenas_stale = True

    def consolidate_weights(self):
        if self._arenas and not self._arenas_stale:
            return
        from .distributed import pack_into_arenas
        flat = {f"{i}/{k}": t for i, d in enumerate(self._weights) for k, t in d.items()}
        if not flat:
            return
        self._arenas, views = pack_into_arenas(flat)
        for name, v in views.items():
            i, k = name.split("/", 1)
            self._weights[int(i)][k] = v
        for i, d in enumerate(self._weights):
            for slot, t in d.items():
                L.call("mvd_engine_set_weight", self._h, i, slot.encode(), _ptr(t), t.numel(), L.dtype_code(t))
        self._arenas_stale = False

    def weight_bytes(self) -> int:
        return sum(t.numel() * t.element_size() for d in self._weights for t in d.values())

    def _ensure_workspace(self, batch, h, w, text_len, ref_batch, keep_features, lay=ViewLayout()):
        key = (batch, h, w, text_len, ref_batch, keep_features) + (() if lay.views else (0,)) + lay.key()
        if self._ws_key == key and not self._ws_resize:
            return
        keep_bound = self._ws_key == key
        self._ws_args = (batch, h, w, text_len, ref_batch, keep_features, lay)
        if lay.rows:
            a = L.mvd_forward_args_t()
            a.batch, a.height, a.width, a.text_len, a.ref_batch, a.views = batch, h, w, text_len, ref_batch, lay.views
            a.cam_rows, a.cam_batch = 4, lay.rows
            a.flags = L.MVD_USE_CAMERA | L.MVD_USE_IMAGE | L.MVD_SHARE_REF
            suffix, beside = self._entry(lay)
            ws = getattr(L.lib(), "mvd_engine_workspace_bytes" + (suffix or "_args"))(self._h, C.byref(a), *beside)
        else:
            ws = L.lib().mvd_engine_workspace_bytes(self._h, batch, h, w, text_len, ref_batch)
        if ws < 0:
            raise L.MvdError(f"workspace_bytes: {L.last_error()}")
        rc = 0
        if ref_batch > 0:
            rc = L.lib().mvd_engine_refcache_bytes(self._h, ref_batch, h, w, int(keep_features))
            if rc < 0:
                raise L.MvdError(f"refcache_bytes: {L.last_error()}")
        self._ws_resize = False
        if keep_bound and self._ws is not None and self._ws.numel() >= ws:
            return
        if self._ws is None or self._ws.numel() < ws:
            self._ws = None
            self._ws = torch.empty(ws, dtype=torch.uint8, device=self.device)
        if rc and (self._rc is None or self._rc.numel() < rc):
# ... 282 lines not shown
```

mvd_amd/ops.py:

```python
from __future__ import annotations

import ctypes as C
from typing import Optional

import torch

from . import _lib as L


def _p(t: Optional[torch.Tensor]):
    if t is None:
        return None
    assert t.is_cuda and t.is_contiguous(), "ops expect contiguous CUDA tensors"
    return C.c_void_p(t.data_ptr())


_s = L.stream


def _bf16(*ts):
    for t in ts:
        if t is not None:
            assert t.dtype == torch.bfloat16, "expected bf16"

# ... 443 lines not shown
    B, hw, c0 = x.shape
    c1 = x2.shape[2] if x2 is not None else 0
    y = torch.empty(B, hw, c0 + c1, device=x.device, dtype=torch.bfloat16)
    ws = torch.empty(B * 256 * groups * 2, device=x.device, dtype=torch.float32)
    L.call("mvd_op_groupnorm", _p(x), _p(x2), c0, c1, B, hw, groups, float(eps), _p(gamma), _p(beta), int(silu), _p(y),
           _p(ws), _s())
    return y


def layernorm(x, gamma, beta, eps=1e-5):
    _bf16(x)
    rows, c = x.shape
    y = torch.empty_like(x)
    L.call("mvd_op_layernorm", _p(x), rows, c, float(eps), _p(gamma), _p(beta), _p(y), _s())
    return y


def refnorm(x):
    _bf16(x)
    B, hw, c = x.shape
    y = torch.empty_like(x)
    L.call("mvd_op_refnorm", _p(x), B, hw, c, _p(y), _s())
    return y


def refnorm_grouped(x, group):
    _bf16(x)
    B, hw, c = x.shape
    y = torch.empty_like(x)
    L.call("mvd_op_refnorm_grouped", _p(x), B, int(group), hw, c, _p(y), _s())
    return y


def film(x, scale, shift):
    _bf16(x)
    B, hw, c = x.shape
    y = torch.empty_like(x)
    L.call("mvd_op_film", _p(x), B, hw, c, _p(scale), _p(shift), _p(y), _s())
    return y


def conv_in(x, w, bias):
    B, H, W, cin = x.shape
    cout = w.shape[0]
    y = torch.empty(B, H, W, cout, device=x.device, dtype=torch.bfloat16)
    L.call("mvd_op_conv_in", _p(x), B, H, W, cin, _p(w), _p(bias), cout, _p(y), _s())
    return y


def conv_out(x, w, bias):
    B, H, W, c = x.shape
    cout = w.shape[0]
    y = torch.empty(B, cout, H, W, device=x.device, dtype=torch.float32)
    L.call("mvd_op_conv_out", _p(x), B, H, W, c, _p(w), _p(bias), cout, _p(y), _s())
    return y


def softmax_rows(s):
    assert s.dtype == torch.float32 and s.dim() == 2
    out = torch.empty(s.shape, device=s.device, dtype=torch.bfloat16)
    L.call("mvd_op_softmax_rows", _p(s), s.shape[0], s.shape[1], _p(out), _s())
    return out


def vae_pointwise(x, w, bias):
    assert x.dtype == torch.float32 and x.dim() == 3 and w.dtype == torch.float32 and w.shape[1] == x.shape[1] and bias.shape == w.shape[:1]
    B, cin, hw = x.shape
    y = torch.empty(B, w.shape[0], hw, device=x.device, dtype=torch.float32)
    L.call("mvd_op_vae_pointwise", _p(x), B, cin, w.shape[0], hw, _p(w), _p(bias), _p(y), _s())
    return y


def _f32(*ts):
    for t in ts:
        if t is not None:
            assert t.dtype == torch.float32, "expected fp32"


def clip_add_ln(x, delta, gamma, beta, eps=1e-5, out_f32=False, tower="text", rows=None, out=None):
    _f32(x, delta, gamma, beta)
    R, H = x.shape
    rows = R if rows is None else rows
    if out is None:
        out = torch.empty(R, H, device=x.device, dtype=torch.float32 if out_f32 else torch.bfloat16)
    assert out.dtype == (torch.float32 if out_f32 else torch.bfloat16) and rows <= R and out.numel() >= rows * H
    assert gamma.shape == (H,) and beta.shape == (H,) and (delta is None or delta.numel() >= rows * H)
    L.call(f"mvd_op_{tower}_add_ln", _p(x), _p(delta), _p(gamma), _p(beta), rows, H, float(eps), None if out_f32 else _p(out),
# ... 444 lines not shown
```

mvd_amd/packing.py:

```python
from __future__ import annotations

from typing import Dict, Optional, Tuple


import torch

from .config import UNetConfig

QSCALE = 64 ** -0.5 * 1.4426950408889634


def _bf(t: torch.Tensor, device) -> torch.Tensor:
    return t.detach().to(device=device, dtype=torch.float32).to(torch.bfloat16).contiguous()


def _f32(t: torch.Tensor, device) -> torch.Tensor:
    return t.detach().to(device=device, dtype=torch.float32).contiguous()


def _conv_w(w: torch.Tensor, tap_major: bool = False) -> torch.Tensor:
    co, ci, kh, kw = w.shape
    w = w.detach().float()
    if tap_major or ci % 64:
        return w.permute(0, 2, 3, 1).reshape(co, kh * kw * ci)
    return w.reshape(co, ci // 64, 64, kh, kw).permute(0, 1, 3, 4, 2).reshape(co, kh * kw * ci)


def block_weight(w: torch.Tensor) -> torch.Tensor:
    n, k = w.shape
    assert n % 32 == 0 and k % 64 == 0, (n, k)
    b = w.reshape(n // 32, 32, k // 64, 8, 8).permute(0, 2, 1, 3, 4)
    r = torch.arange(32, device=w.device)
    slot = torch.arange(8, device=w.device)
    src = slot[None, :] ^ ((r[:, None] >> 1) & 7)
    idx = src[None, None, :, :, None].expand(n // 32, k // 64, 32, 8, 8)
    return torch.gather(b, 3, idx).contiguous().reshape(n, k)


def _geglu_rows(w: torch.Tensor) -> torch.Tensor:
    half = w.shape[0] // 2
    val, gate = w[:half], w[half:]
    rest = w.shape[1:]
    v = val.reshape(half // 16, 1, 16, *rest)
    g = gate.reshape(half // 16, 1, 16, *rest)
    return torch.cat([v, g], dim=1).reshape(w.shape)


XS_K = 320


def _xs_row_perm(device) -> torch.Tensor:
    m = torch.arange(32, device=device)
    return 16 * ((m >> 2) & 1) + 4 * (m >> 3) + (m & 3)


def pack_xs(w: torch.Tensor, bias, geglu: bool = False, device=None) -> torch.Tensor:
    device = device if device is not None else w.device
    w = w.detach().to(device=device, dtype=torch.float32)
# ... 177 lines not shown
                                     (f"{key}.ff1", ff1_w, ff1_b, 3)):
                out[f"{slot}.wf"], out[f"{slot}.cf"] = fold_layernorm(w, f(f"{b}.norm{i}.weight"), f(f"{b}.norm{i}.bias"), bias, device)
        if C == XS_K:
            out[f"{key}.proj_in.wx"] = pack_xs(f(f"{key}.proj_in.weight"), f(f"{key}.proj_in.bias"), device=device)
            if not fold_tail:
                out[f"{key}.proj_out.wx"] = pack_xs(f(f"{key}.proj_out.weight"), f(f"{key}.proj_out.bias"), device=device)
            for a in ("attn1", "attn2"):
                out[f"{key}.{a}.out.wx"] = pack_xs(f(f"{b}.{a}.to_out.0.weight"), f(f"{b}.{a}.to_out.0.bias"), device=device)
            if adapter:
                out[f"{key}.ref_kv.wx"] = pack_xs(out[f"{key}.ref_kv.w"].float(), None, device=device)
            for slot, geglu in ((f"{key}.attn1.qkv", False), (f"{key}.attn2.q", False), (f"{key}.ff1", True)):
                wf, cf = out[f"{slot}.wf"].float(), out[f"{slot}.cf"]
                if geglu:
                    inv = torch.argsort(_geglu_rows(torch.arange(wf.shape[0], device=wf.device)))
                    wf, cf = wf[inv], cf[:, inv]
                out[f"{slot}.wx"] = pack_xs(wf, cf[1], geglu=geglu, device=device)

    out["text_kv.w"] = _bf(torch.cat(tkv, 0), device)
    n = cfg.num_levels
    for i in range(n - 1):
        out[f"down_blocks.{i}.down.w"] = _bf(_conv_w(sd[f"down_blocks.{i}.downsamplers.0.conv.weight"]), device)
        out[f"down_blocks.{i}.down.b"] = _f32(sd[f"down_blocks.{i}.downsamplers.0.conv.bias"], device)
        out[f"up_blocks.{i}.up.w"] = _bf(_conv_w(sd[f"up_blocks.{i}.upsamplers.0.conv.weight"]), device)
        wu = sd[f"up_blocks.{i}.upsamplers.0.conv.weight"]
        if small_batch_twins and wu.shape[0] > cfg.block_out_channels[0] and wu.shape[0] % 128 == 0 and wu.shape[1] % 128 == 0:
            out[f"up_blocks.{i}.up.ws"] = pack_ws(wu, None, device)
        if wu.shape[1] % 64 == 0:
            out[f"up_blocks.{i}.up.w4"] = pack_up4(wu, device)
        out[f"up_blocks.{i}.up.b"] = _f32(sd[f"up_blocks.{i}.upsamplers.0.conv.bias"], device)
    out["conv_norm_out.g"] = _f32(sd["conv_norm_out.weight"], device)
    out["conv_norm_out.b"] = _f32(sd["conv_norm_out.bias"], device)
    out["conv_out.w"] = _bf(_conv_w(sd["conv_out.weight"], tap_major=True), device)
    out["conv_out.b"] = _f32(sd["conv_out.bias"], device)
    return out


def pack_camera(sd: Dict[str, torch.Tensor], device, num_levels: int = 4) -> Dict[str, torch.Tensor]:
    out = {f"cam.{k}": _f32(v, device) for k, v in sd.items()}
    names = [f"down_{i}" for i in range(num_levels)] + [f"up_{i}" for i in range(num_levels)] + ["output"]
    keys = [f"modulators.{n}.{j}.{t}" for n in names for j in (0, 1, 3) for t in ("weight", "bias")]
    if all(k in sd for k in keys):
        cat = lambda j, t: torch.cat([sd[f"modulators.{n}.{j}.{t}"].detach().float() for n in names], 0)
        out["cam.modcat.w0"], out["cam.modcat.b0"] = _f32(cat(0, "weight"), device), _f32(cat(0, "bias"), device)
        out["cam.modcat.g1"], out["cam.modcat.be1"] = _f32(cat(1, "weight"), device), _f32(cat(1, "bias"), device)
        out["cam.modcat.w3"], out["cam.modcat.b3"] = _f32(cat(3, "weight"), device), _f32(cat(3, "bias"), device)
    return out


VGG16_CONVS = ((0, 3, 64), (2, 64, 64), (5, 64, 128), (7, 128, 128), (10, 128, 256), (12, 256, 256), (14, 256, 256),
               (17, 256, 512), (19, 512, 512), (21, 512, 512), (24, 512, 512), (26, 512, 512), (28, 512, 512))
VGG16_POOLS = (4, 9, 16, 23)
VGG16_PARAMS = 14_714_688


def normalize_vgg_keys(sd) -> Dict[str, torch.Tensor]:
    from ._lib import MvdError
    if not hasattr(sd, "keys"):
        raise MvdError(f"VGG-16 weights: expected a state dict, got {type(sd).__name__}")
    out = {}
    for idx, cin, cout in VGG16_CONVS:
        for leaf, shape in (("weight", (cout, cin, 3, 3)), ("bias", (cout,))):
            t = sd.get(f"features.{idx}.{leaf}", sd.get(f"{idx}.{leaf}"))
            if t is None:
                raise MvdError(f"VGG-16 weights: key 'features.{idx}.{leaf}' (or '{idx}.{leaf}') is missing")
            if not isinstance(t, torch.Tensor) or tuple(t.shape) != shape:
                raise MvdError(f"VGG-16 weights: 'features.{idx}.{leaf}' has shape {tuple(getattr(t, 'shape', ()))}, expected {shape}")
# ... 302 lines not shown
```

Baseline: 543.2 forward-passes/s.

## Fuse refnorm into ref_kv GEMM, add MFMA conv_out, cache encoder time projection

After: 548.0 forward-passes/s, median of 6. No clear change (+0.9%).

```diff
diff --git a/include/mvd_hip.h b/include/mvd_hip.h
--- a/include/mvd_hip.h
+++ b/include/mvd_hip.h
@@ -34,6 +34,7 @@
 
 int mvd_engine_set_weight(mvd_engine_t* e, int set, const char* slot, const void* ptr, int64_t numel, int dtype);
 int mvd_engine_clear_weights(mvd_engine_t* e, int set);
+int mvd_engine_weights_written(mvd_engine_t* e);
 
 int64_t mvd_engine_workspace_bytes(mvd_engine_t* e, int batch, int height, int width, int text_len, int ref_batch);
 int64_t mvd_engine_refcache_bytes(mvd_engine_t* e, int ref_batch, int height, int width, int keep_features);
@@ -122,6 +123,8 @@
                      void* out, int m, int n, void* stream);
 int mvd_op_linear_xs(const void* x, int ldx, const void* w_packed, int m, int k, int units, int geglu, int ln, float ln_eps,
                      const void* res, int ldres, void* out, int ldo, int csplit, void* stream);
+int mvd_op_linear_xs_affine(const void* x, int ldx, const void* w_packed, int m, int k, int units, const float* mean_k, int hw,
+                            int group, void* out, int ldo, int csplit, void* stream);
 int mvd_op_conv3x3_ws(const void* x, int batch, int h, int w, int c, const void* w_packed, const float* bias, const float* rowvec,
                       int ld_rowvec, const void* res, const void* sc, const void* sc2, int sc_c1, int sc_c2, void* out, int n,
                       int variant, void* stream);
@@ -147,11 +150,14 @@
                      void* stream);
 int mvd_op_refnorm(const void* x, int batch, int hw, int c, void* y, void* stream);
 int mvd_op_refnorm_grouped(const void* x, int batch, int group, int hw, int c, void* y, void* stream);
+int mvd_op_refnorm_stats(const void* x, int batch, int group, int hw, int c, float* mean_k, void* stream);
 int mvd_op_film(const void* x, int batch, int hw, int c, const float* scale, const float* shift, void* y, void* stream);
 int mvd_op_conv_in(const void* x, int batch, int h, int w, int cin, const float* wt, const float* bias, int cout, void* y,
                    void* stream);
 int mvd_op_conv_out(const void* x, int batch, int h, int w, int c, const void* wt, const float* bias, int cout, float* y,
                     void* stream);
+int mvd_op_conv_out_mfma(const void* x, int batch, int h, int w, int c, const void* wm, const float* bias, int cout, float* y,
+                         void* stream);
 int mvd_op_nchw_to_nhwc(const float* x, int batch, int c, int hw, const float* scale, const float* shift, void* y,
                         void* stream);
 int mvd_op_nhwc_to_nchw(const void* x, int batch, int hw, int c, float* y, void* stream);
@@ -235,6 +241,10 @@
   MVD_DBG_FORK_LATE = 4194304,
   MVD_DBG_SKINNY_VECTOR = 8388608
 } mvd_debug_flag_t;
+enum {
+  MVD_DBG_REFNORM_UNFUSED = 16777216,
+  MVD_DBG_CONV_OUT_SCALAR = 33554432
+};
 int mvd_debug_set_flags(int flags);
 
 int mvd_op_ddpm_step(const float* model_out, const float* sample, const float* noise, float c0, float c1, float c2,
diff --git a/mvd_amd/_lib.py b/mvd_amd/_lib.py
--- a/mvd_amd/_lib.py
+++ b/mvd_amd/_lib.py
@@ -90,6 +90,7 @@
     "mvd_engine_create": (C.c_int, [C.POINTER(mvd_config_t), C.POINTER(C.c_void_p)]),
     "mvd_engine_destroy": (C.c_int, [C.c_void_p]),
     "mvd_engine_set_weight": (C.c_int, [C.c_void_p, C.c_int, C.c_char_p, C.c_void_p, C.c_int64, C.c_int]),
+    "mvd_engine_weights_written": (C.c_int, [C.c_void_p]),
     "mvd_engine_clear_weights": (C.c_int, [C.c_void_p, C.c_int]),
     "mvd_engine_workspace_bytes": (C.c_int64, [C.c_void_p, C.c_int, C.c_int, C.c_int, C.c_int, C.c_int]),
     "mvd_engine_workspace_bytes_args": (C.c_int64, [C.c_void_p, C.POINTER(mvd_forward_args_t)]),
@@ -128,6 +129,8 @@
                                    C.c_int, C.c_int, C.c_void_p]),
     "mvd_op_linear_xs": (C.c_int, [C.c_void_p, C.c_int, C.c_void_p, C.c_int, C.c_int, C.c_int, C.c_int, C.c_int, C.c_float,
                                    C.c_void_p, C.c_int, C.c_void_p, C.c_int, C.c_int, C.c_void_p]),
+    "mvd_op_linear_xs_affine": (C.c_int, [C.c_void_p, C.c_int, C.c_void_p, C.c_int, C.c_int, C.c_int, C.c_void_p, C.c_int, C.c_int,
+                                          C.c_void_p, C.c_int, C.c_int, C.c_void_p]),
     "mvd_op_conv3x3_ws": (C.c_int, [C.c_void_p, C.c_int, C.c_int, C.c_int, C.c_int, C.c_void_p, C.c_void_p, C.c_void_p, C.c_int,
                                     C.c_void_p, C.c_void_p, C.c_void_p, C.c_int, C.c_int, C.c_void_p, C.c_int, C.c_int, C.c_void_p]),
     "mvd_op_conv3x3": (C.c_int, [C.c_void_p, C.c_int, C.c_int, C.c_int, C.c_int, C.c_int, C.c_int, C.c_int, C.c_void_p, C.c_void_p,
@@ -156,8 +159,10 @@
     "mvd_op_layernorm": (C.c_int, [C.c_void_p, C.c_int, C.c_int, C.c_float, C.c_void_p, C.c_void_p, C.c_void_p, C.c_void_p]),
     "mvd_op_refnorm": (C.c_int, [C.c_void_p, C.c_int, C.c_int, C.c_int, C.c_void_p, C.c_void_p]),
     "mvd_op_refnorm_grouped": (C.c_int, [C.c_void_p, C.c_int, C.c_int, C.c_int, C.c_int, C.c_void_p, C.c_void_p]),
+    "mvd_op_refnorm_stats": (C.c_int, [C.c_void_p, C.c_int, C.c_int, C.c_int, C.c_int, C.c_void_p, C.c_void_p]),
     "mvd_op_film": (C.c_int, [C.c_void_p, C.c_int, C.c_int, C.c_int, C.c_void_p, C.c_void_p, C.c_void_p, C.c_void_p]),
     "mvd_op_conv_in": (C.c_int, [C.c_void_p, C.c_int, C.c_int, C.c_int, C.c_int, C.c_void_p, C.c_void_p, C.c_int, C.c_void_p, C.c_void_p]),
+    "mvd_op_conv_out_mfma": (C.c_int, [C.c_void_p, C.c_int, C.c_int, C.c_int, C.c_int, C.c_void_p, C.c_void_p, C.c_int, C.c_void_p, C.c_void_p]),
     "mvd_op_conv_out": (C.c_int, [C.c_void_p, C.c_int, C.c_int, C.c_int, C.c_int, C.c_void_p, C.c_void_p, C.c_int, C.c_void_p, C.c_void_p]),
     "mvd_op_nchw_to_nhwc": (C.c_int, [C.c_void_p, C.c_int, C.c_int, C.c_int, C.c_void_p, C.c_void_p, C.c_void_p, C.c_void_p]),
     "mvd_op_nhwc_to_nchw": (C.c_int, [C.c_void_p, C.c_int, C.c_int, C.c_int, C.c_void_p, C.c_void_p]),
diff --git a/mvd_amd/csrc/engine.hip b/mvd_amd/csrc/engine.hip
--- a/mvd_amd/csrc/engine.hip
+++ b/mvd_amd/csrc/engine.hip
@@ -63,6 +63,8 @@
   bool dc_on = false; int dc_branch = 0;
   void* dc_ptr = nullptr; int64_t dc_bytes = 0;
   uint64_t weight_gen = 0;
+  float* enc_tp = nullptr; size_t enc_tp_cap = 0;
+  bool enc_tp_valid = false; int enc_tp_set = 0, enc_tp_batch = 0; uint64_t enc_tp_wgen = 0;
   struct DeepRecord { bool valid = false; int batch = 0, h = 0, w = 0, cam = 0, img = 0, branch = 0; uint64_t wgen = 0; std::vector<int> layout; } dc_rec;
   bool dc_sizing = false;
   int dc_hidden_channels() const { return cfg.layers_per_block - 1 - dc_branch >= 1 ? cfg.block_out_channels[0] : cfg.block_out_channels[1]; }
@@ -92,6 +94,7 @@
   ~mvd_engine() {
     drop_graphs();
     for (auto& sl : kv_slots) if (sl.dev) (void)hipFree(sl.dev);
+    if (enc_tp) (void)hipFree(enc_tp);
     for (hipEvent_t ev : ev_pool) (void)hipEventDestroy(ev);
     for (hipEvent_t ev : feat_ev) if (ev) (void)hipEventDestroy(ev);
     if (fork_ev) (void)hipEventDestroy(fork_ev);
@@ -265,16 +268,18 @@
   }
 
   int try_xs(const bf16_t* x, int K, int M, const std::string& slot, int64_t n_full, int N, bool geglu, bool ln,
-             const bf16_t* res, int ldres, void* out, int ldo, int set_override = -1) {
+             const bf16_t* res, int ldres, void* out, int ldo, int set_override = -1, const float* aff = nullptr, int aff_hw = 0,
+             int aff_span = 0, bool probe = false) {
     if (err) return err;
     if (dry || (g_debug_flags & MVD_DBG_NO_XS) || K != 320 || slot.empty() || !has(slot, set_override)) return 0;
     MvdXsArgs a; memset(&a, 0, sizeof(a));
     a.x = x; a.ldx = K; a.M = M; a.K = K; a.units = N / 32; a.geglu = geglu; a.ln = ln; a.ln_eps = 1e-5f;
-    a.res = res; a.ldres = ldres; a.out = (bf16_t*)out; a.ldo = ldo;
+    a.res = res; a.ldres = ldres; a.out = (bf16_t*)out; a.ldo = ldo; a.aff = aff; a.aff_hw = aff_hw; a.aff_span = aff_span;
     if (N % 64 || !mvd_gemm_xs_applicable(a)) return 0;
     if ((long)((M + 255) / 256) * mvd_gemm_xs_pick_csplit(a) < 448) return 0;
     a.w = WB(slot, (n_full / 32) * 21 * 512, set_override);
     if (!a.w) return err;
+    if (probe) return 1;
     e->prof_M = M; e->prof_N = N; e->prof_K = K; e->prof_tag = geglu * 10 + (ln ? 1 : 0);
     const int r = profiled(geglu ? MVD_PC_XS_GEGLU : (res ? MVD_PC_XS_RESIDUAL : (ln ? MVD_PC_XS_LN_DENSE : MVD_PC_XS_DENSE)), 2.0 * M * (double)N * K, 0.0, [&] { return mvd_launch_gemm_xs(a, s); });
     return r ? r : 1;
@@ -589,12 +594,26 @@
     if (o.capture) {
       const size_t mk = c.e->tmp.off;
       bf16_t* rn = c.talloc<bf16_t>((size_t)M * C);
+      float* rmk = c.talloc<float>((size_t)2 * M);
       if (o.defer_norm) {
         if (!c.dry && !c.err) CHECK(mvd_launch_refstats(out.p, B_, hw, C, o.stats + 2 * c.e->feat_pixel_off(feat_idx), c.s));
       } else {
-        if (!c.dry && !c.err) CHECK(o.layout->per_object_stats() ? mvd_launch_refnorm_grouped(out.p, B_, 1, hw, C, rn, c.s) : mvd_launch_refnorm(out.p, B_, hw, C, rn, c.s));
-        CHECK(c.linear(rn, nullptr, C, 0, M, c.WB(key + ".ref_kv.w", (int64_t)4 * C * C, 0), nullptr, 4 * C, nullptr, 0, c.e->refkv[feat_idx], 4 * C, false, false, 0,
-                       key + ".ref_kv.wx", 0));
+        const int grp = o.layout->per_object_stats() ? 1 : B_;
+        int fused = 0;
+        if (!c.dry && !c.err && !(g_debug_flags & MVD_DBG_REFNORM_UNFUSED)) {
+          fused = c.try_xs(out.p, C, M, key + ".ref_kv.wx", (int64_t)4 * C, 4 * C, false, false, nullptr, 0, c.e->refkv[feat_idx], 4 * C, 0, rmk, hw, grp * hw, true);
+          if (fused < 0) return fused;
+        }
+        if (fused) {
+          CHECK(mvd_launch_refnorm_stats(out.p, B_, grp, hw, C, rmk, c.s));
+          const int r = c.try_xs(out.p, C, M, key + ".ref_kv.wx", (int64_t)4 * C, 4 * C, false, false, nullptr, 0, c.e->refkv[feat_idx], 4 * C, 0, rmk, hw, grp * hw);
+          if (r < 0) return r;
+          if (r != 1) { mvd_set_error("forward: the row-affine ref_kv launch of %s was refused after its probe", key.c_str()); return c.err = -16; }
+        } else {
+          if (!c.dry && !c.err) CHECK(o.layout->per_object_stats() ? mvd_launch_refnorm_grouped(out.p, B_, 1, hw, C, rn, c.s) : mvd_launch_refnorm(out.p, B_, hw, C, rn, c.s));
+          CHECK(c.linear(rn, nullptr, C, 0, M, c.WB(key + ".ref_kv.w", (int64_t)4 * C * C, 0), nullptr, 4 * C, nullptr, 0, c.e->refkv[feat_idx], 4 * C, false, false, 0,
+                         key + ".ref_kv.wx", 0));
+        }
         if (c.e->dual_now && !c.dry && !c.err && hipEventRecord(c.e->feat_ev[feat_idx], c.s) != hipSuccess) { mvd_set_error("forward: hipEventRecord failed"); return -3; }
       }
       if (c.e->rc_keep && !c.dry && !c.err)
@@ -718,13 +737,17 @@
       CHECK(c.groupnorm(h.p, nullptr, C0, 0, B, h.hw(), cfg.norm_eps, c.WF("conv_norm_out.g", C0), c.WF("conv_norm_out.b", C0), 1, t.p));
       const bf16_t* wo = c.WB("conv_out.w", (int64_t)cfg.out_channels * 9 * C0);
       const float* bo = c.WF("conv_out.b", cfg.out_channels);
-      if (!c.dry && !c.err) CHECK(mvd_launch_conv_out(t.p, B, h.H, h.W, C0, wo, bo, cfg.out_channels, out_nchw, c.s));
+      if (!c.dry && !c.err && c.has("conv_out.wm") && !(g_debug_flags & MVD_DBG_CONV_OUT_SCALAR) &&
+          mvd_conv_out_mfma_applicable(B, h.H, h.W, C0, cfg.out_channels)) {
+        const bf16_t* wm = c.WB("conv_out.wm", mvd_conv_out_mfma_packed_elems(C0, cfg.out_channels));
+        if (!c.err) CHECK(mvd_launch_conv_out_mfma(t.p, B, h.H, h.W, C0, wm, bo, cfg.out_channels, out_nchw, c.s));
+      } else if (!c.dry && !c.err) CHECK(mvd_launch_conv_out(t.p, B, h.H, h.W, C0, wo, bo, cfg.out_channels, out_nchw, c.s));
     }
     return c.err;
   }
 };
 
-int time_path(Ctx& c, const float* timesteps, int B, const float** tproj_out) {
+int time_path(Ctx& c, const float* timesteps, int B, const float** tproj_out, bool launch = true) {
   const mvd_config_t& cfg = c.e->cfg;
   const int C0 = cfg.block_out_channels[0], TD = 4 * C0;
   float* sinus = c.talloc<float>((size_t)B * C0);
@@ -740,12 +763,36 @@
   const float* bp = c.WF("temb_proj.b", c.e->temb_total);
   *tproj_out = tproj;
   if (c.err) return c.err;
-  if (c.dry) return 0;
+  if (c.dry || !launch) return 0;
   CHECK(mvd_launch_timestep_embedding(timesteps, B, C0, sinus, c.s));
   CHECK(mvd_launch_skinny_linear(sinus, C0, B, C0, w1, 1, b1, TD, 0, t1, TD, c.s));
   CHECK(mvd_launch_skinny_linear(t1, TD, B, TD, w2, 1, b2, TD, 1, emb, TD, c.s));
   CHECK(mvd_launch_silu_to_bf16(emb, (int64_t)B * TD, act, c.s));
   CHECK(c.linear(act, nullptr, TD, 0, B, wp, bp, c.e->temb_total, nullptr, 0, tproj, c.e->temb_total, false, true));
+  return 0;
+}
+
+int encoder_time_path(Ctx& c, float* tz, int Br, const float** tproj_out) {
+  mvd_engine* e = c.e;
+  const bool hit = !c.dry && !e->prof && e->enc_tp && e->enc_tp_valid && e->enc_tp_set == c.set && e->enc_tp_batch == Br && e->enc_tp_wgen == e->weight_gen;
+  if (!c.dry && !hit && !c.err) CHECK((int)hipMemsetAsync(tz, 0, Br * sizeof(float), c.s));
+  const float* arena = nullptr;
+  CHECK(time_path(c, tz, Br, &arena, !hit));
+  *tproj_out = hit ? e->enc_tp : arena;
+  if (c.dry || hit || c.err || e->prof) return c.err;
+  hipStreamCaptureStatus cs = hipStreamCaptureStatusNone;
+  if (c.s && (hipStreamIsCapturing(c.s, &cs) != hipSuccess || cs != hipStreamCaptureStatusNone)) return 0;
+  const size_t bytes = (size_t)Br * e->temb_total * sizeof(float);
+  if (e->enc_tp) e->drop_graphs();
+  e->enc_tp_valid = false;
+  if (e->enc_tp_cap < bytes) {
+    if (e->enc_tp) (void)hipFree(e->enc_tp);
+    e->enc_tp = nullptr; e->enc_tp_cap = 0;
+    if (hipMalloc((void**)&e->enc_tp, bytes) != hipSuccess) { mvd_set_error("forward: hipMalloc of the encoder's time projection failed"); return -3; }
+    e->enc_tp_cap = bytes;
+  }
+  if (hipMemcpyAsync(e->enc_tp, arena, bytes, hipMemcpyDeviceToDevice, c.s) != hipSuccess) { mvd_set_error("forward: copy of the encoder's time projection failed"); return -3; }
+  e->enc_tp_valid = true; e->enc_tp_set = c.set; e->enc_tp_batch = Br; e->enc_tp_wgen = e->weight_gen;
   return 0;
 }
 
@@ -990,8 +1037,7 @@
     CHECK(time_path(c, a.timesteps, B, &tproj_main));
     c.set = e->share_encoder ? 0 : 1;
     float* tz = c.aalloc<float>(a.ref_batch);
-    if (!dry) CHECK((int)hipMemsetAsync(tz, 0, a.ref_batch * sizeof(float), s));
-    CHECK(time_path(c, tz, a.ref_batch, &tproj_enc));
+    CHECK(encoder_time_path(c, tz, a.ref_batch, &tproj_enc));
     c.set = 0;
     CHECK(fork());
   }
@@ -1005,8 +1051,7 @@
     const float* tproj = tproj_enc;
     if (!tproj) {
       float* tz = c.talloc<float>(Br);
-      if (!dry) CHECK((int)hipMemsetAsync(tz, 0, Br * sizeof(float), c.s));
-      CHECK(time_path(c, tz, Br, &tproj));
+      CHECK(encoder_time_path(c, tz, Br, &tproj));
     }
     bf16_t* tx = c.aalloc<bf16_t>((size_t)Br * L * xd);
     Act xin = c.new_act(Br, H, Wd, 64, true);
@@ -1134,6 +1179,12 @@
   if (!e || set < 0 || set > 1 || !slot || !ptr || numel <= 0 || dtype < 0 || dtype > 1) { mvd_set_error("set_weight: bad argument"); return -1; }
   if ((uintptr_t)ptr & 15) { mvd_set_error("set_weight: '%s' must be 16-byte aligned", slot); return -1; }
   e->w[set].m[slot] = Weight{ptr, numel, dtype};
+  ++e->weight_gen;
+  return 0;
+}
+int mvd_engine_weights_written(mvd_engine_t* e) {
+  if (!e) { mvd_set_error("weights_written: null engine"); return -1; }
+  e->drop_graphs();
   ++e->weight_gen;
   return 0;
 }
@@ -1862,11 +1913,17 @@
 int mvd_op_refnorm_grouped(const void* x, int batch, int group, int hw, int c, void* y, void* stream) {
   return mvd_launch_refnorm_grouped((const bf16_t*)x, batch, group, hw, c, (bf16_t*)y, (hipStream_t)stream);
 }
+int mvd_op_refnorm_stats(const void* x, int batch, int group, int hw, int c, float* mean_k, void* stream) {
+  return mvd_launch_refnorm_stats((const bf16_t*)x, batch, group, hw, c, mean_k, (hipStream_t)stream);
+}
 int mvd_op_film(const void* x, int batch, int hw, int c, const float* scale, const float* shift, void* y, void* stream) {
   return mvd_launch_film((const bf16_t*)x, batch, hw, c, scale, shift, c, (bf16_t*)y, (hipStream_t)stream);
 }
 int mvd_op_conv_in(const void* x, int batch, int h, int w, int cin, const float* wt, const float* bias, int cout, void* y, void* stream) {
   return mvd_launch_conv_in((const bf16_t*)x, batch, h, w, cin, wt, bias, cout, (bf16_t*)y, (hipStream_t)stream);
+}
+int mvd_op_conv_out_mfma(const void* x, int batch, int h, int w, int c, const void* wm, const float* bias, int cout, float* y, void* stream) {
+  return mvd_launch_conv_out_mfma((const bf16_t*)x, batch, h, w, c, (const bf16_t*)wm, bias, cout, y, (hipStream_t)stream);
 }
 int mvd_op_conv_out(const void* x, int batch, int h, int w, int c, const void* wt, const float* bias, int cout, float* y, void* stream) {
   return mvd_launch_conv_out((const bf16_t*)x, batch, h, w, c, (const bf16_t*)wt, bias, cout, y, (hipStream_t)stream);
diff --git a/mvd_amd/csrc/gemm_xs.hip b/mvd_amd/csrc/gemm_xs.hip
--- a/mvd_amd/csrc/gemm_xs.hip
+++ b/mvd_amd/csrc/gemm_xs.hip
@@ -9,13 +9,13 @@
 
 #define XS_WAIT_VM(n) asm volatile("s_waitcnt vmcnt(" #n ")" ::: "memory")
 
-template <int KS, bool GEGLU, bool RES, bool LN>
+template <int KS, bool GEGLU, bool RES, bool LN, bool AFF = false>
 __global__ __launch_bounds__(256, 2) void gemm_xs_kernel(const MvdXsArgs a) {
   constexpr int NW = 4, RT = 2, NS = GEGLU ? 2 : 3;
   constexpr int STG = GEGLU ? 8192 : 4096;
   constexpr int UNIT = (KS + 1) * 1024;
   constexpr int P = KS / NW;
-  static_assert(KS % NW == 0 && !(GEGLU && RES) && !(RES && LN), "shape of the instantiations");
+  static_assert(KS % NW == 0 && !(GEGLU && RES) && !(RES && LN) && !(AFF && (GEGLU || RES || LN)), "shape of the instantiations");
   constexpr int E = 2 * RT + (RES ? 2 * RT : 0);
   extern __shared__ __attribute__((aligned(16))) unsigned char smem[];
   const int lane = threadIdx.x & 63;
@@ -51,6 +51,15 @@
   if (NS == 3 && nit > 1) issue_unit(1, 1);
 
   const __amdgpu_buffer_rsrc_t rs_x = buf_rsrc(a.x, (int)((size_t)a.M * a.ldx * 2));
+  float aff_m[RT], aff_k[RT];
+  if constexpr (AFF) {
+#pragma unroll
+    for (int t = 0; t < RT; ++t) {
+      const int row = min(row_w + t * 32 + r, a.M - 1);
+      const float* mk = a.aff + 2 * ((size_t)(row / a.aff_span) * a.aff_hw + row % a.aff_hw);
+      aff_m[t] = mk[0]; aff_k[t] = mk[1];
+    }
+  }
   u32x4 x[RT][KS];
 #pragma unroll
   for (int t = 0; t < RT; ++t) {
@@ -83,6 +92,18 @@
         const unsigned d[4] = {x[t][s].x, x[t][s].y, x[t][s].z, x[t][s].w};
         x[t][s] = u32x4{pack2bf(fmaf(bflo(d[0]), rstd, nb), fmaf(bfhi(d[0]), rstd, nb)), pack2bf(fmaf(bflo(d[1]), rstd, nb), fmaf(bfhi(d[1]), rstd, nb)),
                         pack2bf(fmaf(bflo(d[2]), rstd, nb), fmaf(bfhi(d[2]), rstd, nb)), pack2bf(fmaf(bflo(d[3]), rstd, nb), fmaf(bfhi(d[3]), rstd, nb))};
+      }
+    }
+  }
+  if constexpr (AFF) {
+#pragma unroll
+    for (int t = 0; t < RT; ++t) {
+      const float mean = aff_m[t], k = aff_k[t];
+#pragma unroll
+      for (int s = 0; s < KS; ++s) {
+        const unsigned d[4] = {x[t][s].x, x[t][s].y, x[t][s].z, x[t][s].w};
+        x[t][s] = u32x4{pack2bf((bflo(d[0]) - mean) * k, (bfhi(d[0]) - mean) * k), pack2bf((bflo(d[1]) - mean) * k, (bfhi(d[1]) - mean) * k),
+                        pack2bf((bflo(d[2]) - mean) * k, (bfhi(d[2]) - mean) * k), pack2bf((bflo(d[3]) - mean) * k, (bfhi(d[3]) - mean) * k)};
       }
     }
   }
@@ -292,26 +313,26 @@
 #endif
 }
 
-template <int KS, bool GEGLU, bool RES, bool LN>
+template <int KS, bool GEGLU, bool RES, bool LN, bool AFF = false>
 int launch_xs(const MvdXsArgs& a, hipStream_t s) {
   constexpr int LDS_BYTES = (GEGLU ? 2 : 3) * (KS + 1) * 1024 + 4 * (GEGLU ? 8192 : 4096);
   static bool init[16] = {};
   int dev = 0;
   (void)hipGetDevice(&dev);
   if (!init[dev & 15]) {
-    hipError_t e = hipFuncSetAttribute(reinterpret_cast<const void*>(&gemm_xs_kernel<KS, GEGLU, RES, LN>), hipFuncAttributeMaxDynamicSharedMemorySize, LDS_BYTES);
+    hipError_t e = hipFuncSetAttribute(reinterpret_cast<const void*>(&gemm_xs_kernel<KS, GEGLU, RES, LN, AFF>), hipFuncAttributeMaxDynamicSharedMemorySize, LDS_BYTES);
     if (e != hipSuccess) { mvd_set_error("gemm_xs: hipFuncSetAttribute: %s", hipGetErrorString(e)); return -2; }
     init[dev & 15] = true;
     if (MVD_ENV_INT("MVD_XS_TRACE", 0)) {
       int occ = -1;
-      (void)hipOccupancyMaxActiveBlocksPerMultiprocessor(&occ, reinterpret_cast<const void*>(&gemm_xs_kernel<KS, GEGLU, RES, LN>), 256, LDS_BYTES);
+      (void)hipOccupancyMaxActiveBlocksPerMultiprocessor(&occ, reinterpret_cast<const void*>(&gemm_xs_kernel<KS, GEGLU, RES, LN, AFF>), 256, LDS_BYTES);
       fprintf(stderr, "gemm_xs<%d,%d,%d,%d>: %d workgroups per CU by the occupancy query (LDS %d B)\n", KS, (int)GEGLU, (int)RES, (int)LN, occ, LDS_BYTES);
     }
   }
   const int nrb = (a.M + 255) / 256;
   const int grid = a.csplit == 1 ? nrb : ((nrb + 7) / 8) * 8 * a.csplit;
   g_mvd_last_gemm.cfg = 9; g_mvd_last_gemm.splitk = 1; g_mvd_last_gemm.tiles = nrb * a.csplit; g_mvd_last_gemm.grid = grid; g_mvd_last_gemm.per_cu = 2;
-  hipLaunchKernelGGL((gemm_xs_kernel<KS, GEGLU, RES, LN>), dim3(grid), dim3(256), LDS_BYTES, s, a);
+  hipLaunchKernelGGL((gemm_xs_kernel<KS, GEGLU, RES, LN, AFF>), dim3(grid), dim3(256), LDS_BYTES, s, a);
   hipError_t e = hipGetLastError();
   if (e != hipSuccess) { mvd_set_error("gemm_xs launch: %s", hipGetErrorString(e)); return -3; }
   return 0;
@@ -324,6 +345,7 @@
   if (a.K != 320 || a.units <= 0 || a.M <= 0 || a.relu) return false;
   if (a.units % (a.geglu ? 4 : 2)) return false;
   if ((a.geglu || a.ln) && a.res) return false;
+  if (a.aff && (a.geglu || a.ln || a.res || a.aff_hw <= 0 || a.aff_span < a.aff_hw || a.aff_span % a.aff_hw)) return false;
   if ((size_t)(a.M + 256) * a.ldx * 2 >= lim || (size_t)(a.M + 256) * a.ldo * 2 >= lim) return false;
   if (a.res && (size_t)(a.M + 256) * a.ldres * 2 >= lim) return false;
   if ((size_t)a.units * 21 * 1024 >= lim) return false;
@@ -349,6 +371,7 @@
   }
   if (a.geglu) return a.ln ? launch_xs<20, true, false, true>(a, s) : launch_xs<20, true, false, false>(a, s);
   if (a.res) return launch_xs<20, false, true, false>(a, s);
+  if (a.aff) return launch_xs<20, false, false, false, true>(a, s);
   return a.ln ? launch_xs<20, false, false, true>(a, s) : launch_xs<20, false, false, false>(a, s);
 }
 
@@ -360,3 +383,13 @@
   if (!x || !w_packed || !out) { mvd_set_error("mvd_op_linear_xs: null operand"); return -1; }
   return mvd_launch_gemm_xs(a, (hipStream_t)stream);
 }
+
+extern "C" int mvd_op_linear_xs_affine(const void* x, int ldx, const void* w_packed, int m, int k, int units, const float* mean_k,
+                                       int hw, int group, void* out, int ldo, int csplit, void* stream) {
+  MvdXsArgs a; memset(&a, 0, sizeof(a));
+  a.x = (const bf16_t*)x; a.ldx = ldx; a.w = (const bf16_t*)w_packed; a.M = m; a.K = k; a.units = units;
+  a.out = (bf16_t*)out; a.ldo = ldo; a.csplit = csplit; a.aff = mean_k; a.aff_hw = hw; a.aff_span = group * hw;
+  if (!x || !w_packed || !out || !mean_k) { mvd_set_error("mvd_op_linear_xs_affine: null operand"); return -1; }
+  if (hw <= 0 || group <= 0 || m % (group * hw)) { mvd_set_error("mvd_op_linear_xs_affine: %d rows are not whole groups of %d maps of %d pixels", m, group, hw); return -1; }
+  return mvd_launch_gemm_xs(a, (hipStream_t)stream);
+}
diff --git a/mvd_amd/csrc/kernels.h b/mvd_amd/csrc/kernels.h
--- a/mvd_amd/csrc/kernels.h
+++ b/mvd_amd/csrc/kernels.h
@@ -78,6 +78,7 @@
   bf16_t* out; int ldo;
   int csplit;
   int relu;
+  const float* aff; int aff_hw, aff_span;
 };
 bool mvd_gemm_xs_applicable(const MvdXsArgs& a);
 int mvd_gemm_xs_pick_csplit(const MvdXsArgs& a);
@@ -136,6 +137,7 @@
                          bf16_t* y, hipStream_t s);
 int mvd_launch_refnorm(const bf16_t* x, int batch, int hw, int c, bf16_t* y, hipStream_t s);
 int mvd_launch_refnorm_grouped(const bf16_t* x, int batch, int group, int hw, int c, bf16_t* y, hipStream_t s);
+int mvd_launch_refnorm_stats(const bf16_t* x, int batch, int group, int hw, int c, float* mean_k , hipStream_t s);
 int mvd_launch_refstats(const bf16_t* x, int batch, int hw, int c, float* stats , hipStream_t s);
 int mvd_launch_refapply(const bf16_t* x, int batch, int hw, int c, const float* mean_k , bf16_t* y, hipStream_t s);
 
@@ -147,6 +149,10 @@
                      bf16_t* skip_out, hipStream_t stream);
 int mvd_launch_conv_in(const bf16_t* x, int batch, int h, int w, int cin, const float* wt, const float* bias,
                        int cout, bf16_t* y, hipStream_t s);
+bool mvd_conv_out_mfma_applicable(int batch, int h, int w, int c, int cout);
+int64_t mvd_conv_out_mfma_packed_elems(int c, int cout);
+int mvd_launch_conv_out_mfma(const bf16_t* x, int batch, int h, int w, int c, const bf16_t* wm, const float* bias, int cout,
+                             float* y, hipStream_t s);
 int mvd_launch_conv_out(const bf16_t* x, int batch, int h, int w, int c, const bf16_t* wt, const float* bias,
                         int cout, float* y, hipStream_t s);
 int mvd_launch_im2col_in(const float* x, int batch, int c, int h, int w, const float* scale, const float* shift, int ld_ss,
diff --git a/mvd_amd/csrc/misc.hip b/mvd_amd/csrc/misc.hip
--- a/mvd_amd/csrc/misc.hip
+++ b/mvd_amd/csrc/misc.hip
@@ -2,6 +2,7 @@
 #include <stdio.h>
 #include <stdlib.h>
 #include "host_util.h"
+#include "bufaddr.h"
 
 static thread_local char g_err[512] = "";
 void mvd_set_error(const char* fmt, ...) {
@@ -120,6 +121,63 @@
     if (co < cout) {
       const float t = wave_sum(acc[co]);
       if (lane == 0) y[((size_t)b * cout + co) * hw + p] = t + bias[co];
+    }
+  }
+}
+
+template <int R>
+__global__ __launch_bounds__(256) void conv_out_mfma_kernel(const bf16_t* __restrict__ x, int batch, int h, int w, int c,
+                                                             const bf16_t* __restrict__ wm, const float* __restrict__ bias,
+                                                             int cout, float* __restrict__ y, int ngroups, int gpr) {
+  extern __shared__ __attribute__((aligned(16))) unsigned char conv_out_smem[];
+  constexpr int U = 5;
+  const int ncs = c >> 5;
+  const int frag = 4 * R * 16;
+  {
+    const int n16 = 9 * ncs * 4 * R;
+    const u32x4* src = reinterpret_cast<const u32x4*>(wm);
+    u32x4* dst = reinterpret_cast<u32x4*>(conv_out_smem);
+    for (int i = threadIdx.x; i < n16; i += 256) dst[i] = src[i];
+  }
+  __syncthreads();
+  const int lane = threadIdx.x & 63, wave = threadIdx.x >> 6;
+  const int col = lane & 15, kg = lane >> 4;
+  const __amdgpu_buffer_rsrc_t rs = buf_rsrc(x, (int)((size_t)batch * h * w * c * 2));
+  const bool arow = col < R;
+  const unsigned char* ap = conv_out_smem + (kg * R + (col & (R - 1))) * 16;
+  const u32x4 zero4 = {0u, 0u, 0u, 0u};
+  const size_t hw = (size_t)h * w;
+  for (int g = blockIdx.x * 4 + wave; g < ngroups; g += gridDim.x * 4) {
+    const int gx = g % gpr, row = g / gpr;
+    const int oy = row % h, b = row / h;
+    const int ox = gx * 16 + col;
+    f32x4 acc[2] = {{0.f, 0.f, 0.f, 0.f}, {0.f, 0.f, 0.f, 0.f}};
+#pragma unroll
+    for (int tap = 0; tap < 9; ++tap) {
+      const int dy = tap / 3 - 1, dx = tap % 3 - 1;
+      const int iy = oy + dy, ix = ox + dx;
+      const bool ok = (unsigned)iy < (unsigned)h && (unsigned)ix < (unsigned)w && ox < w;
+      const unsigned vo = ok ? (unsigned)(((row + dy) * w + ix) * c * 2 + kg * 16) : OOB;
+      for (int cs0 = 0; cs0 < ncs; cs0 += U) {
+        u32x4 xv[U];
+#pragma unroll
+        for (int u = 0; u < U; ++u) xv[u] = cs0 + u < ncs ? __builtin_amdgcn_raw_buffer_load_b128(rs, (int)(vo + (unsigned)(cs0 + u) * 64u), 0, 0) : zero4;
+#pragma unroll
+        for (int u = 0; u < U; ++u) {
+          if (cs0 + u < ncs) {
+            const u32x4 lw = *reinterpret_cast<const u32x4*>(ap + (tap * ncs + cs0 + u) * frag);
+            const u32x4 av = arow ? lw : zero4;
+            acc[u & 1] = __builtin_amdgcn_mfma_f32_16x16x32_bf16(__builtin_bit_cast(bf16x8, av), __builtin_bit_cast(bf16x8, xv[u]), acc[u & 1], 0, 0, 0);
+          }
+        }
+      }
+    }
+    if (ox < w) {
+#pragma unroll
+      for (int i = 0; i < 4; ++i) {
+        const int ch = kg * 4 + i;
+        if (ch < cout) y[((size_t)b * cout + ch) * hw + (size_t)oy * w + ox] = (acc[0][i] + acc[1][i]) + bias[ch];
+      }
     }
   }
 }
@@ -510,6 +568,26 @@
   return launch_check("conv_out");
 }
 
+bool mvd_conv_out_mfma_applicable(int batch, int h, int w, int c, int cout) {
+  if (batch <= 0 || h <= 0 || w <= 0 || c <= 0 || (c % 32) || cout <= 0 || cout > 8) return false;
+  if ((size_t)batch * h * w * c * 2 >= ((size_t)1 << 31) || (size_t)batch * h >= ((size_t)1 << 26)) return false;
+  return (size_t)9 * c * (cout <= 4 ? 4 : 8) * 2 <= 65536;
+}
+int64_t mvd_conv_out_mfma_packed_elems(int c, int cout) { return (int64_t)9 * c * (cout <= 4 ? 4 : 8); }
+
+int mvd_launch_conv_out_mfma(const bf16_t* x, int batch, int h, int w, int c, const bf16_t* wm, const float* bias, int cout,
+                             float* y, hipStream_t s) {
+  if (!x || !y || !wm || !bias || !mvd_conv_out_mfma_applicable(batch, h, w, c, cout)) { mvd_set_error("conv_out_mfma: bad arguments or not a shape of the kernel (C %% 32, cout <= 8)"); return -1; }
+  const int gpr = (w + 15) / 16, ngroups = batch * h * gpr;
+  const int R = cout <= 4 ? 4 : 8;
+  const size_t lds = (size_t)9 * c * R * 2;
+  int grid = nblk(ngroups, 4);
+  if (grid > 512) grid = 512;
+  if (R == 4) hipLaunchKernelGGL(conv_out_mfma_kernel<4>, dim3(grid), dim3(256), lds, s, x, batch, h, w, c, wm, bias, cout, y, ngroups, gpr);
+  else hipLaunchKernelGGL(conv_out_mfma_kernel<8>, dim3(grid), dim3(256), lds, s, x, batch, h, w, c, wm, bias, cout, y, ngroups, gpr);
+  return launch_check("conv_out_mfma");
+}
+
 int mvd_launch_f32_to_bf16(const float* x, int64_t n, bf16_t* y, hipStream_t s) {
   if (!x || !y || n <= 0) { mvd_set_error("f32_to_bf16: bad arguments"); return -1; }
   int grid = nblk(n, 256);
diff --git a/mvd_amd/csrc/norm.hip b/mvd_amd/csrc/norm.hip
--- a/mvd_amd/csrc/norm.hip
+++ b/mvd_amd/csrc/norm.hip
@@ -403,6 +403,114 @@
     for (int j = 0; j < 8; ++j) f[j] = (f[j] - mean) * k;
     *reinterpret_cast<u32x4*>(y + off) = pack8(f);
   }
+}
+
+template <int NV, bool STATS>
+__global__ __launch_bounds__(256) void refnorm_reg_kernel(const bf16_t* __restrict__ x, int group, int hw, int c,
+                                                          bf16_t* __restrict__ y, float* __restrict__ mean_k) {
+  __shared__ float red[8];
+  const int p = blockIdx.x;
+  const size_t base = (size_t)blockIdx.y * group * hw * c;
+  x += base;
+  const int vec = c >> 3;
+  const int total = group * vec;
+  const int lane = threadIdx.x & 63, wave = threadIdx.x >> 6;
+  auto block_sum = [&](float v) -> float {
+    v = wave_sum(v);
+    __syncthreads();
+    if (lane == 0) red[wave] = v;
+    __syncthreads();
+    return red[0] + red[1] + red[2] + red[3];
+  };
+  u32x4 v[NV];
+  unsigned off[NV];
+#pragma unroll
+  for (int i = 0; i < NV; ++i) {
+    const int e = threadIdx.x + i * 256;
+    v[i] = u32x4{0u, 0u, 0u, 0u}; off[i] = 0u;
+    if (e < total) {
+      const int b = e / vec, vv = e % vec;
+      off[i] = ((unsigned)b * hw + p) * c + vv * 8;
+      v[i] = *reinterpret_cast<const u32x4*>(x + off[i]);
+    }
+  }
+  float s = 0.f;
+#pragma unroll
+  for (int i = 0; i < NV; ++i) {
+    if (threadIdx.x + i * 256 < total) {
+      float f[8];
+      unpack8(v[i], f);
+#pragma unroll
+      for (int j = 0; j < 8; ++j) s += f[j];
+    }
+  }
+  const float n = (float)group * (float)c;
+  const float mean = block_sum(s) / n;
+  float q = 0.f;
+#pragma unroll
+  for (int i = 0; i < NV; ++i) {
+    if (threadIdx.x + i * 256 < total) {
+      float f[8];
+      unpack8(v[i], f);
+#pragma unroll
+      for (int j = 0; j < 8; ++j) { const float d = f[j] - mean; q = fmaf(d, d, q); }
+    }
+  }
+  const float var = block_sum(q) / (n - 1.0f);
+  const float k = 0.5f / fmaxf(sqrtf(var), 1e-6f);
+  if constexpr (STATS) {
+    if (threadIdx.x == 0) { float* o = mean_k + 2 * ((size_t)blockIdx.y * hw + p); o[0] = mean; o[1] = k; }
+  } else {
+    y += base;
+#pragma unroll
+    for (int i = 0; i < NV; ++i) {
+      if (threadIdx.x + i * 256 < total) {
+        float f[8];
+        unpack8(v[i], f);
+#pragma unroll
+        for (int j = 0; j < 8; ++j) f[j] = (f[j] - mean) * k;
+        *reinterpret_cast<u32x4*>(y + off[i]) = pack8(f);
+      }
+    }
+  }
+}
+
+__global__ __launch_bounds__(256) void refnorm_stats_loop_kernel(const bf16_t* __restrict__ x, int group, int hw, int c,
+                                                                 float* __restrict__ mean_k) {
+  __shared__ float red[8];
+  const int p = blockIdx.x;
+  x += (size_t)blockIdx.y * group * hw * c;
+  const int vec = c >> 3;
+  const int total = group * vec;
+  const int lane = threadIdx.x & 63, wave = threadIdx.x >> 6;
+  auto block_sum = [&](float v) -> float {
+    v = wave_sum(v);
+    __syncthreads();
+    if (lane == 0) red[wave] = v;
+    __syncthreads();
+    return red[0] + red[1] + red[2] + red[3];
+  };
+  float s = 0.f;
+  for (int e = threadIdx.x; e < total; e += 256) {
+    const int b = e / vec, v = e % vec;
+    float f[8];
+    unpack8(*reinterpret_cast<const u32x4*>(x + ((size_t)b * hw + p) * c + v * 8), f);
+#pragma unroll
+    for (int j = 0; j < 8; ++j) s += f[j];
+  }
+  const float n = (float)group * (float)c;
+  const float mean = block_sum(s) / n;
+  float q = 0.f;
+  for (int e = threadIdx.x; e < total; e += 256) {
+    const int b = e / vec, v = e % vec;
+    float f[8];
+    unpack8(*reinterpret_cast<const u32x4*>(x + ((size_t)b * hw + p) * c + v * 8), f);
+#pragma unroll
+    for (int j = 0; j < 8; ++j) { const float d = f[j] - mean; q = fmaf(d, d, q); }
+  }
+  const float var = block_sum(q) / (n - 1.0f);
+  const float k = 0.5f / fmaxf(sqrtf(var), 1e-6f);
+  if (threadIdx.x == 0) { float* o = mean_k + 2 * ((size_t)blockIdx.y * hw + p); o[0] = mean; o[1] = k; }
 }
 
 __global__ __launch_bounds__(256) void refstats_kernel(const bf16_t* __restrict__ x, int batch, int hw, int c, float* __restrict__ stats) {
@@ -592,9 +700,23 @@
   hipLaunchKernelGGL(refapply_kernel, dim3((unsigned)grid), dim3(256), 0, s, x, batch, hw, c, mean_k, y);
   return check_launch("refapply");
 }
+template <bool STATS>
+static bool launch_refnorm_reg(const bf16_t* x, int batch, int group, int hw, int c, bf16_t* y, float* mean_k, hipStream_t s) {
+  if (mvd_debug_flags() & MVD_DBG_REFNORM_UNFUSED) return false;
+  const long total = (long)group * (c >> 3);
+  const long nv = (total + 255) / 256;
+  if (nv > 20 || (long)group * hw * c >= (1L << 31)) return false;
+  const dim3 grid(hw, batch / group), blk(256);
+#define REFNORM_REG(NVT) hipLaunchKernelGGL((refnorm_reg_kernel<NVT, STATS>), grid, blk, 0, s, x, group, hw, c, y, mean_k)
+  if (nv <= 1) REFNORM_REG(1); else if (nv <= 2) REFNORM_REG(2); else if (nv <= 5) REFNORM_REG(5); else if (nv <= 10) REFNORM_REG(10); else REFNORM_REG(20);
+#undef REFNORM_REG
+  return true;
+}
+
 int mvd_launch_refnorm(const bf16_t* x, int batch, int hw, int c, bf16_t* y, hipStream_t s) {
   if (!x || !y || batch <= 0 || hw <= 0 || c <= 0 || (c % 8)) { mvd_set_error("refnorm: bad arguments"); return -1; }
-  hipLaunchKernelGGL(refnorm_kernel, dim3(hw), dim3(256), 0, s, x, batch, hw, c, y);
+  if (!launch_refnorm_reg<false>(x, batch, batch, hw, c, y, nullptr, s))
+    hipLaunchKernelGGL(refnorm_kernel, dim3(hw), dim3(256), 0, s, x, batch, hw, c, y);
   return check_launch("refnorm");
 }
 
@@ -602,8 +724,18 @@
   if (!x || !y || batch <= 0 || hw <= 0 || c <= 0 || (c % 8)) { mvd_set_error("refnorm_grouped: bad arguments"); return -1; }
   if (group <= 0 || batch % group) { mvd_set_error("refnorm_grouped: group %d does not divide the batch %d", group, batch); return -1; }
   if (batch / group > 65535) { mvd_set_error("refnorm_grouped: %d groups exceed the grid", batch / group); return -1; }
-  hipLaunchKernelGGL(refnorm_grouped_kernel, dim3(hw, batch / group), dim3(256), 0, s, x, group, hw, c, y);
+  if (!launch_refnorm_reg<false>(x, batch, group, hw, c, y, nullptr, s))
+    hipLaunchKernelGGL(refnorm_grouped_kernel, dim3(hw, batch / group), dim3(256), 0, s, x, group, hw, c, y);
   return check_launch("refnorm_grouped");
+}
+
+int mvd_launch_refnorm_stats(const bf16_t* x, int batch, int group, int hw, int c, float* mean_k, hipStream_t s) {
+  if (!x || !mean_k || batch <= 0 || hw <= 0 || c <= 0 || (c % 8)) { mvd_set_error("refnorm_stats: bad arguments"); return -1; }
+  if (group <= 0 || batch % group) { mvd_set_error("refnorm_stats: group %d does not divide the batch %d", group, batch); return -1; }
+  if (batch / group > 65535) { mvd_set_error("refnorm_stats: %d groups exceed the grid", batch / group); return -1; }
+  if (!launch_refnorm_reg<true>(x, batch, group, hw, c, nullptr, mean_k, s))
+    hipLaunchKernelGGL(refnorm_stats_loop_kernel, dim3(hw, batch / group), dim3(256), 0, s, x, group, hw, c, mean_k);
+  return check_launch("refnorm_stats");
 }
 
 int mvd_launch_layernorm_f32(const float* x, int rows, int c, float eps, const float* gamma, const float* beta, int silu,
diff --git a/mvd_amd/distributed.py b/mvd_amd/distributed.py
--- a/mvd_amd/distributed.py
+++ b/mvd_amd/distributed.py
@@ -133,7 +133,11 @@
     if not dist.is_initialized() or dist.get_world_size() == 1:
         return dict(bytes=0, seconds=0.0, buckets=0)
     engine.consolidate_weights()
-    return broadcast_arenas(engine._arenas.values(), src, bucket_bytes)
+    stats = broadcast_arenas(engine._arenas.values(), src, bucket_bytes)
+    written = getattr(engine, "weights_written", None)
+    if written is not None:
+        written()
+    return stats
 
 
 def merge_reference_stats(local: torch.Tensor, group=None) -> torch.Tensor:
diff --git a/mvd_amd/engine.py b/mvd_amd/engine.py
--- a/mvd_amd/engine.py
+++ b/mvd_amd/engine.py
@@ -102,6 +102,9 @@
             for slot, t in d.items():
                 L.call("mvd_engine_set_weight", self._h, i, slot.encode(), _ptr(t), t.numel(), L.dtype_code(t))
         self._arenas_stale = False
+
+    def weights_written(self):
+        L.call("mvd_engine_weights_written", self._h)
 
     def weight_bytes(self) -> int:
         return sum(t.numel() * t.element_size() for d in self._weights for t in d.values())
diff --git a/mvd_amd/ops.py b/mvd_amd/ops.py
--- a/mvd_amd/ops.py
+++ b/mvd_amd/ops.py
@@ -499,6 +499,26 @@
     return y
 
 
+def refnorm_stats(x, group=None):
+    _bf16(x)
+    B, hw, c = x.shape
+    group = B if group is None else int(group)
+    mk = torch.empty(B // max(group, 1), hw, 2, device=x.device, dtype=torch.float32)
+    L.call("mvd_op_refnorm_stats", _p(x), B, group, hw, c, _p(mk), _s())
+    return mk
+
+
+def linear_xs_affine(x, w_packed, mean_k, hw, group, csplit=0):
+    _bf16(x, w_packed)
+    m, k = x.shape
+    units = w_packed.shape[0]
+    assert x.is_contiguous() and mean_k.dtype == torch.float32 and mean_k.is_contiguous() and mean_k.numel() == 2 * m // group
+    out = torch.empty(m, units * 32, device=x.device, dtype=torch.bfloat16)
+    L.call("mvd_op_linear_xs_affine", _p(x), k, _p(w_packed), m, k, units, _p(mean_k), int(hw), int(group), _p(out), units * 32,
+           csplit, _s())
+    return out
+
+
 def film(x, scale, shift):
     _bf16(x)
     B, hw, c = x.shape
@@ -520,6 +540,16 @@
     cout = w.shape[0]
     y = torch.empty(B, cout, H, W, device=x.device, dtype=torch.float32)
     L.call("mvd_op_conv_out", _p(x), B, H, W, c, _p(w), _p(bias), cout, _p(y), _s())
+    return y
+
+
+def conv_out_mfma(x, wm, bias):
+    _bf16(x, wm)
+    B, H, W, c = x.shape
+    cout = bias.numel()
+    assert wm.is_contiguous() and wm.numel() == 9 * c * (4 if cout <= 4 else 8)
+    y = torch.empty(B, cout, H, W, device=x.device, dtype=torch.float32)
+    L.call("mvd_op_conv_out_mfma", _p(x), B, H, W, c, _p(wm), _p(bias), cout, _p(y), _s())
     return y
 
 
diff --git a/mvd_amd/packing.py b/mvd_amd/packing.py
--- a/mvd_amd/packing.py
+++ b/mvd_amd/packing.py
@@ -24,6 +24,21 @@
     if tap_major or ci % 64:
         return w.permute(0, 2, 3, 1).reshape(co, kh * kw * ci)
     return w.reshape(co, ci // 64, 64, kh, kw).permute(0, 1, 3, 4, 2).reshape(co, kh * kw * ci)
+
+
+def pack_conv_out_mfma(w: torch.Tensor) -> torch.Tensor:
+    co, ci, kh, kw = w.shape
+    assert kh == 3 and kw == 3 and ci % 32 == 0 and 1 <= co <= 8, w.shape
+    r = 4 if co <= 4 else 8
+    t = torch.zeros(r, 9, ci, dtype=torch.float32, device=w.device)
+    t[:co] = w.detach().float().permute(0, 2, 3, 1).reshape(co, 9, ci)
+    return t.view(r, 9, ci // 32, 4, 8).permute(1, 2, 3, 0, 4).contiguous().to(torch.bfloat16)
+
+
+def unpack_conv_out_mfma(wm: torch.Tensor, cout: int) -> torch.Tensor:
+    _nine, ncs, _kg, r, _e = wm.shape
+    t = wm.float().permute(3, 0, 1, 2, 4).reshape(r, 3, 3, ncs * 32)
+    return t[:cout].permute(0, 3, 1, 2).contiguous()
 
 
 def block_weight(w: torch.Tensor) -> torch.Tensor:
@@ -267,6 +282,9 @@
     out["conv_norm_out.b"] = _f32(sd["conv_norm_out.bias"], device)
     out["conv_out.w"] = _bf(_conv_w(sd["conv_out.weight"], tap_major=True), device)
     out["conv_out.b"] = _f32(sd["conv_out.bias"], device)
+    wo = sd["conv_out.weight"]
+    if wo.shape[1] % 32 == 0 and wo.shape[0] <= 8:
+        out["conv_out.wm"] = pack_conv_out_mfma(wo).to(device)
     return out
 
 
```
